# etheriqa/amber

Hardware: AMD Instinct MI355X
Metric: Mrays/sec + wall-clock, Cornell 1024^2 @1024spp; 1/2/4/8 GPU (higher is better)
Workload: dtype f32

## Files before the change

### amber_amd/api.py

```python
from __future__ import annotations

import ctypes as C
import os
import subprocess
from pathlib import Path

import numpy as np

_ROOT = Path(__file__).resolve().parent
_LIB_PATH = _ROOT / "lib" / os.environ.get("AMBER_AMD_LIB", "libamber_hip.so")
_lib = None


class AmberError(RuntimeError):
    """Raised for every non-zero return code of the C ABI (message = amber_hip_last_error())."""


class FlatObject(C.Structure):
    _fields_ = [("kind", C.c_uint32), ("material", C.c_uint32), ("p", C.c_float * 12)]


class FlatMaterial(C.Structure):
    _fields_ = [("kind", C.c_uint32), ("rho", C.c_float * 3), ("param", C.c_float), ("r0", C.c_float)]

# ... 51 lines not shown
class Photon(C.Structure):
    _fields_ = [("pos", C.c_float * 3), ("object", C.c_int32), ("dir_out", C.c_float * 3), ("path", C.c_uint32),
                ("weight", C.c_float * 3), ("sample", C.c_uint32), ("normal", C.c_float * 3), ("bounce", C.c_uint32)]


class PhotonInfo(C.Structure):
    _fields_ = [("n_photons", C.c_uint64), ("n_written", C.c_uint64), ("n_rays", C.c_uint64), ("n_launches", C.c_uint32), ("n_repeats", C.c_uint32)]


class AccumulateInfo(C.Structure):
    _fields_ = [("n_launches", C.c_uint32), ("n_repeats", C.c_uint32), ("rec_count", C.c_uint32), ("flag_words_set", C.c_uint32),
                ("flags_dirty", C.c_uint32)]


LT_SPLAT_CAPACITY0 = 65536
SPLAT_DTYPE = np.dtype([("path", np.uint32), ("sample", np.uint32), ("bounce", np.uint32), ("pixel", np.uint32), ("rgb", np.float32, (3,)), ("pad", np.uint32)])
PHOTON_DIFFUSE, PHOTON_SPECULAR, PHOTON_LIGHT, PHOTON_EYE, PHOTON_ALL = 1, 2, 4, 8, 15
PHOTONS_HOST = 1
PHOTON_CAPACITY0 = 65536
PHOTON_DTYPE = np.dtype([("pos", np.float32, (3,)), ("object", np.int32), ("dir_out", np.float32, (3,)), ("path", np.uint32),
                         ("weight", np.float32, (3,)), ("sample", np.uint32), ("normal", np.float32, (3,)), ("bounce", np.uint32)])


class Ray(C.Structure):
    _fields_ = [("origin", C.c_float * 3), ("t_max", C.c_float), ("dir", C.c_float * 3), ("pad", C.c_uint32)]


class RayHit(C.Structure):
    _fields_ = [("t", C.c_float), ("object", C.c_int32), ("pos", C.c_float * 3), ("normal", C.c_float * 3)]


class PathRay(C.Structure):
    _fields_ = [("origin", C.c_float * 3), ("pad0", C.c_uint32), ("dir", C.c_float * 3), ("pad1", C.c_uint32),
                ("weight", C.c_float * 3), ("pad2", C.c_uint32), ("rng_state", C.c_uint64), ("pad3", C.c_uint64)]


class PathResult(C.Structure):
    _fields_ = [("rgb", C.c_float * 3), ("casts", C.c_uint32), ("rng_state", C.c_uint64), ("pad", C.c_uint32 * 2)]


class AovPixel(C.Structure):
    _fields_ = [("albedo", C.c_float * 3), ("depth", C.c_float), ("normal", C.c_float * 3), ("coverage", C.c_float)]


class DenoiseParams(C.Structure):
    _fields_ = [("levels", C.c_uint32), ("k_normal", C.c_float), ("k_albedo", C.c_float), ("k_depth", C.c_float), ("k_color", C.c_float),
                ("reserved", C.c_uint32 * 3)]


class MomentsPixel(C.Structure):
    _fields_ = [("m1", C.c_float), ("m2", C.c_float), ("batches", C.c_float), ("pad", C.c_float)]


class DenoiseVarianceParams(C.Structure):
    _fields_ = [("levels", C.c_uint32), ("k_normal", C.c_float), ("k_albedo", C.c_float), ("k_depth", C.c_float), ("k_lum", C.c_float),
                ("var_radius", C.c_uint32), ("reserved", C.c_uint32 * 2)]


class TemporalParams(C.Structure):
    _fields_ = [("levels", C.c_uint32), ("max_history", C.c_uint32), ("k_normal", C.c_float), ("k_albedo", C.c_float), ("k_depth", C.c_float),
                ("k_color", C.c_float), ("reserved", C.c_uint32 * 2)]


class HistoryPixel(C.Structure):
    _fields_ = [("color", C.c_float * 3), ("length", C.c_float), ("m1", C.c_float), ("m2", C.c_float), ("pad", C.c_float * 2)]


class BvhDumpInfo(C.Structure):
    _fields_ = [("n_nodes", C.c_uint32), ("n_prims", C.c_uint32), ("root", C.c_int32), ("depth", C.c_uint32),
                ("gmin", C.c_float * 3), ("step", C.c_float * 3), ("reach", C.c_float * 3)]


class HostStats(C.Structure):
    _fields_ = [("rays", C.c_uint64), ("passes", C.c_uint64), ("launches", C.c_uint32), ("pad", C.c_uint32), ("kernel_ms", C.c_double)]


PRIM_TRIANGLE, PRIM_SPHERE, PRIM_DISK, PRIM_CYLINDER = 0, 1, 2, 3
_RECORD = np.dtype([("kind", np.uint32), ("material", np.uint32), ("p", np.float32, (12,))])
MAT_LAMBERTIAN, MAT_PHONG, MAT_SPECULAR, MAT_REFRACTION, MAT_DIFFUSE_LIGHT, MAT_EYE = 0, 1, 2, 3, 4, 5
ENGINE_AUTO, ENGINE_LIST, ENGINE_TWO_PHASE, ENGINE_BVH, ENGINE_WAVEFRONT = 0, 1, 2, 3, 4
ENGINE_REFERENCE_BVH = 6
PT_FLAG_NULL_STREAM, PT_FLAG_BVH_POOL, PT_FLAG_BVH_ITEMS = 1, 2, 4
PT_FLAG_DEVICE_BUILD = 8
BUILD_NONE, BUILD_HOST, BUILD_DEVICE, BUILD_HOST_FALLBACK = 0, 1, 2, 3
BUILD_REASON_NONE, BUILD_REASON_DEPTH, BUILD_REASON_WIDE, BUILD_REASON_BOUNDS = 0, 1, 2, 3
RAYS_HOST = 1
_RAY = np.dtype([("origin", np.float32, (3,)), ("t_max", np.float32), ("dir", np.float32, (3,)), ("pad", np.uint32)])
_RAY_HIT = np.dtype([("t", np.float32), ("object", np.int32), ("pos", np.float32, (3,)), ("normal", np.float32, (3,))])
_PATH_RAY = np.dtype([("origin", np.float32, (3,)), ("pad0", np.uint32), ("dir", np.float32, (3,)), ("pad1", np.uint32),
                      ("weight", np.float32, (3,)), ("pad2", np.uint32), ("rng_state", np.uint64), ("pad3", np.uint64)])
_PATH_RESULT = np.dtype([("rgb", np.float32, (3,)), ("casts", np.uint32), ("rng_state", np.uint64), ("pad", np.uint32, (2,))])
RESOLVE_MEAN_F32, RESOLVE_RGB8, RESOLVE_RGBA8 = 0, 1, 2
RESOLVE_HOST, RESOLVE_MIRROR_X = 1, 2
UPDATE_REFIT, UPDATE_REBUILD = 0, 1

ABI_SYMBOLS = [
    "amber_hip_pt_create", "amber_hip_pt_render_pass", "amber_hip_pt_clear", "amber_hip_pt_sync",
    "amber_hip_pt_download", "amber_hip_pt_device_framebuffer", "amber_hip_pt_stream", "amber_hip_pt_local_rows", "amber_hip_pt_kernel_time", "amber_hip_pt_build_info", "amber_hip_pt_update_objects", "amber_hip_pt_update_lens",
    "amber_hip_pt_cast_rays", "amber_hip_pt_occluded", "amber_hip_pt_resolve", "amber_hip_pt_destroy",
    "amber_hip_pt_trace_paths", "amber_hip_sampler_state",
    "amber_hip_pt_aov_pass", "amber_hip_pt_aov_clear", "amber_hip_pt_aov_download", "amber_hip_pt_device_aov", "amber_hip_pt_denoise",
    "amber_hip_pt_render_batch", "amber_hip_pt_moments_clear", "amber_hip_pt_moments_download", "amber_hip_pt_device_moments", "amber_hip_pt_denoise_variance",
    "amber_hip_pt_temporal", "amber_hip_pt_temporal_reset", "amber_hip_pt_history_download", "amber_hip_pt_device_history",
    "amber_hip_last_error", "amber_hip_abi_version", "amber_hip_math_mode", "amber_hip_device_count", "amber_hip_lt_trace", "amber_hip_lt_trace_range", "amber_hip_lt_render_pass",
    "amber_hip_lt_trace_photons",
    "amber_host_cornell_box", "amber_host_scene_import", "amber_host_scene_create", "amber_host_scene_destroy", "amber_host_scene_flatten",
    "amber_host_pt_create", "amber_host_render", "amber_host_render_devices", "amber_host_last_error", "amber_host_tonemap", "amber_host_export",
]
LAB_SYMBOLS = [
    "amber_hip_kat_cast", "amber_hip_kat_sample", "amber_hip_kat_eye", "amber_hip_kat_trace", "amber_hip_kat_math", "amber_hip_kat_signatures", "amber_hip_pt_signatures",
    "amber_hip_kat_traversal_rate", "amber_hip_kat_pixel_masks", "amber_hip_kat_bvh_dump", "amber_hip_kat_division",
    "amber_hip_kat_sqrt", "amber_hip_kat_sqrt_sweep", "amber_hip_kat_lt_accumulate", "amber_hip_kat_lt_stage_ms",
    "amber_hip_kat_photon_stage_ms",
    "amber_hip_kat_light_ray", "amber_hip_kat_lens_response", "amber_hip_kat_radiance", "amber_host_kat_scene_lights",
    "amber_hip_kat_accumulate", "amber_hip_kat_phase_a",
]
PRODUCT_LIB, LAB_LIB = "libamber_hip.so", "libamber_hip_lab.so"


def library_path() -> Path:
    return _LIB_PATH


def build_library(force: bool = False) -> Path:
    import shutil
    if shutil.which(os.environ.get("HIPCC", "hipcc")) or not _LIB_PATH.exists():
        subprocess.run(["make", "-C", str(_ROOT / "csrc")] + (["-B"] if force else []), check=True)
    return _LIB_PATH


def is_lab() -> bool:
    return hasattr(load_library(), "amber_hip_kat_cast")


def load_library() -> C.CDLL:
    global _lib
    if _lib is not None:
        return _lib
    if not _LIB_PATH.exists():
        raise AmberError(f"{_LIB_PATH} is missing: build it with `make -C amber_amd/csrc` "
                         "(or __graft_entry__.build()); amber_amd has no CPU fallback")
    lib = C.CDLL(str(_LIB_PATH))
    vp, u32, u64, i32 = C.c_void_p, C.c_uint32, C.c_uint64, C.c_int32
    lib.amber_hip_last_error.restype = C.c_char_p
    lib.amber_host_last_error.restype = C.c_char_p
    lib.amber_hip_pt_create.argtypes = [C.POINTER(FlatSceneC), C.POINTER(Sensor), C.POINTER(PtParams), C.POINTER(vp)]
    lib.amber_hip_pt_render_pass.argtypes = [vp, u32, u32]
    lib.amber_hip_pt_clear.argtypes = [vp]
    lib.amber_hip_pt_sync.argtypes = [vp]
    lib.amber_hip_pt_download.argtypes = [vp, vp, C.POINTER(u64)]
    lib.amber_hip_pt_device_framebuffer.argtypes = [vp, C.POINTER(vp), C.POINTER(u64)]
    lib.amber_hip_pt_local_rows.argtypes = [vp, C.POINTER(u32)]
    lib.amber_hip_pt_stream.argtypes = [vp, C.POINTER(vp)]
    lib.amber_hip_pt_kernel_time.argtypes = [vp, C.POINTER(u32), C.POINTER(C.c_double)]
    lib.amber_hip_pt_destroy.argtypes = [vp]
    lib.amber_hip_pt_destroy.restype = None
    if hasattr(lib, "amber_hip_pt_build_info"):
        lib.amber_hip_pt_build_info.argtypes = [vp, C.POINTER(BuildInfo)]
    if hasattr(lib, "amber_hip_pt_update_objects"):
        lib.amber_hip_pt_update_objects.argtypes = [vp, u32, u32, vp, u32, C.POINTER(UpdateInfo)]
    if hasattr(lib, "amber_hip_pt_update_lens"):
        lib.amber_hip_pt_update_lens.argtypes = [vp, C.POINTER(FlatThinLens), vp, u32, C.POINTER(UpdateInfo)]
    if hasattr(lib, "amber_hip_pt_cast_rays"):
        lib.amber_hip_pt_cast_rays.argtypes = [vp, u64, vp, vp, u32]
        lib.amber_hip_pt_occluded.argtypes = [vp, u64, vp, vp, u32]
    if hasattr(lib, "amber_hip_pt_trace_paths"):
        lib.amber_hip_pt_trace_paths.argtypes = [vp, u64, vp, vp, u32, u32, u32]
        lib.amber_hip_sampler_state.argtypes = [u64, u32, u32]
        lib.amber_hip_sampler_state.restype = u64
    if hasattr(lib, "amber_hip_pt_resolve"):
        lib.amber_hip_pt_resolve.argtypes = [vp, u32, u32, vp, u64, u32]
    if hasattr(lib, "amber_hip_pt_aov_pass"):
        lib.amber_hip_pt_aov_pass.argtypes = [vp, u32, u32]
        lib.amber_hip_pt_aov_clear.argtypes = [vp]
        lib.amber_hip_pt_aov_download.argtypes = [vp, vp]
        lib.amber_hip_pt_device_aov.argtypes = [vp, C.POINTER(vp), C.POINTER(u64)]
    if hasattr(lib, "amber_hip_pt_denoise"):
        lib.amber_hip_pt_denoise.argtypes = [vp, u32, C.POINTER(DenoiseParams), u32, vp, u64, u32]
    if hasattr(lib, "amber_hip_pt_render_batch"):
        lib.amber_hip_pt_render_batch.argtypes = [vp, u32, u32]
        lib.amber_hip_pt_moments_clear.argtypes = [vp]
        lib.amber_hip_pt_moments_download.argtypes = [vp, vp]
        lib.amber_hip_pt_device_moments.argtypes = [vp, C.POINTER(vp), C.POINTER(u64)]
        lib.amber_hip_pt_denoise_variance.argtypes = [vp, u32, C.POINTER(DenoiseVarianceParams), u32, vp, u64, u32]
    if hasattr(lib, "amber_hip_pt_temporal"):
        lib.amber_hip_pt_temporal.argtypes = [vp, u32, C.POINTER(TemporalParams), u32, vp, u64, u32]
        lib.amber_hip_pt_temporal_reset.argtypes = [vp]
        lib.amber_hip_pt_history_download.argtypes = [vp, vp]
        lib.amber_hip_pt_device_history.argtypes = [vp, C.POINTER(vp), C.POINTER(u64)]
    if hasattr(lib, "amber_hip_lt_trace"):
        lib.amber_hip_lt_trace.argtypes = [vp, u32, u32, vp, u32, C.POINTER(u32), C.POINTER(u64)]
    if hasattr(lib, "amber_hip_lt_trace_range"):
        lib.amber_hip_lt_trace_range.argtypes = [vp, u32, u32, u32, u32, vp, u32, C.POINTER(u32), C.POINTER(u64)]
    if hasattr(lib, "amber_hip_lt_render_pass"):
        lib.amber_hip_lt_render_pass.argtypes = [vp, u32, u32, C.POINTER(LtPassInfo)]
        if hasattr(lib, "amber_hip_lt_trace_photons"):
            lib.amber_hip_lt_trace_photons.argtypes = [vp, u32, u32, u32, u32, u32, vp, u64, C.POINTER(PhotonInfo), u32]
        if hasattr(lib, "amber_hip_kat_photon_stage_ms"):
            lib.amber_hip_kat_photon_stage_ms.argtypes = [vp, C.POINTER(C.c_double), C.POINTER(C.c_double), C.POINTER(C.c_double)]
    if hasattr(lib, "amber_hip_kat_cast"):
        if hasattr(lib, "amber_hip_kat_phase_a"):
            lib.amber_hip_kat_phase_a.argtypes = [vp, u32, vp, vp, i32, vp, u64, C.POINTER(C.c_uint32)]
        lib.amber_hip_kat_cast.argtypes = [vp, u32, vp, vp, vp, vp, vp, vp]
        lib.amber_hip_kat_sample.argtypes = [vp, u32, vp, vp, vp, vp, vp, vp]
        lib.amber_hip_kat_eye.argtypes = [vp, u32, vp, vp, vp]
        lib.amber_hip_kat_trace.argtypes = [vp, u32, vp, vp, u32, vp, vp]
        lib.amber_hip_kat_math.argtypes = [i32, i32, u32, vp, vp]
        lib.amber_hip_kat_signatures.argtypes = [vp, u32, u32, vp]
        lib.amber_hip_kat_pixel_masks.argtypes = [vp, vp, vp, C.POINTER(C.c_uint32), C.POINTER(C.c_double)]
        lib.amber_hip_kat_traversal_rate.argtypes = [vp, u32, vp, vp, u32, u32, u32, vp, vp, C.POINTER(C.c_double), vp]
        lib.amber_hip_pt_signatures.argtypes = [vp, u32, u32, vp]
        lib.amber_hip_kat_bvh_dump.argtypes = [vp, vp, u32, vp, u32, C.POINTER(BvhDumpInfo)]
        if hasattr(lib, "amber_hip_kat_division"):
            lib.amber_hip_kat_division.argtypes = [i32, i32, u32, vp, vp]
        if hasattr(lib, "amber_hip_kat_sqrt"):
            lib.amber_hip_kat_sqrt.argtypes = [i32, i32, u32, vp, vp]
            lib.amber_hip_kat_sqrt_sweep.argtypes = [i32, u32, u64, C.POINTER(SqrtSweep)]
        if hasattr(lib, "amber_hip_kat_lt_accumulate"):
            lib.amber_hip_kat_lt_accumulate.argtypes = [vp, vp, u32]
            lib.amber_hip_kat_lt_stage_ms.argtypes = [vp, C.POINTER(C.c_double), C.POINTER(C.c_double)]
        if hasattr(lib, "amber_hip_kat_light_ray"):
            lib.amber_hip_kat_light_ray.argtypes = [vp, u32, vp, vp, vp, vp, vp]
            lib.amber_hip_kat_lens_response.argtypes = [vp, u32, vp, vp, vp, vp, vp]
            lib.amber_hip_kat_radiance.argtypes = [vp, u32, vp, vp, vp, vp]
            lib.amber_host_kat_scene_lights.argtypes = [vp, C.POINTER(FlatLight), C.POINTER(u32)]
        if hasattr(lib, "amber_hip_kat_accumulate"):
            lib.amber_hip_kat_accumulate.argtypes = [vp, u32, vp, vp, u32, u32, u32, u64, C.POINTER(AccumulateInfo)]
    lib.amber_host_cornell_box.restype = vp
    lib.amber_host_cornell_box.argtypes = [C.c_float, C.c_float, u32]
    lib.amber_host_scene_import.restype = vp
    lib.amber_host_scene_import.argtypes = [C.c_char_p]
    lib.amber_host_scene_create.restype = vp
    lib.amber_host_scene_create.argtypes = [C.POINTER(FlatObject), u32, C.POINTER(FlatMaterial), u32, C.POINTER(C.c_float),
                                            C.c_float, C.c_float, C.c_float, u32, C.c_int]
    lib.amber_host_scene_destroy.argtypes = [vp]
    lib.amber_host_scene_destroy.restype = None
    lib.amber_host_scene_flatten.argtypes = [vp, C.POINTER(FlatObject), C.POINTER(u32), C.POINTER(FlatMaterial), C.POINTER(u32),
                                             C.POINTER(FlatThinLens)]
    lib.amber_host_pt_create.argtypes = [vp, C.POINTER(Sensor), C.POINTER(PtParams), C.POINTER(vp)]
    lib.amber_host_render.argtypes = [vp, C.c_char_p, C.POINTER(Sensor), u32, u64, u32, C.c_int, u32, vp, C.POINTER(HostStats)]
    lib.amber_host_render_devices.argtypes = [vp, C.c_char_p, C.POINTER(Sensor), u32, u64, u32, C.POINTER(C.c_int), u32, u32, vp, C.POINTER(HostStats)]
    lib.amber_host_tonemap.argtypes = [vp, u32, u32, vp]
    lib.amber_host_export.argtypes = [vp, u32, u32, C.c_char_p, C.c_char_p]
    _lib = lib
    return lib


def _check(rc: int, host: bool = False) -> None:
    if rc != 0:
        lib = load_library()
        msg = (lib.amber_host_last_error() if host else lib.amber_hip_last_error()) or b""
        if host and not msg:
            msg = lib.amber_hip_last_error() or b""
        raise AmberError(f"amber error {rc}: {msg.decode(errors='replace')}")


def device_count() -> int:
    return int(load_library().amber_hip_device_count())


def _f32(a) -> np.ndarray:
    return np.ascontiguousarray(a, dtype=np.float32)


class HostScene:

    def __init__(self, handle):
        if not handle:
            raise AmberError("scene creation failed: " + (load_library().amber_host_last_error() or b"").decode())
        self._h = C.c_void_p(handle)

    @classmethod
    def cornell_box(cls, focal_length: float = 0.050, aperture_radius: float = 0.050, n_blades: int = 6) -> "HostScene":
        return cls(load_library().amber_host_cornell_box(focal_length, aperture_radius, n_blades))

    @classmethod
    def import_file(cls, filename) -> "HostScene":
        return cls(load_library().amber_host_scene_import(str(filename).encode()))

    @classmethod
    def create(cls, objects, materials, transform, focal_length, focus_distance, radius, n_blades, accel: int = 0) -> "HostScene":
        objs = (FlatObject * max(1, len(objects)))()
        for i, (kind, mat, params) in enumerate(objects):
            objs[i].kind, objs[i].material = kind, mat
            for j, v in enumerate(params):
                objs[i].p[j] = v
        mats = (FlatMaterial * max(1, len(materials)))()
        for i, (kind, rho, param) in enumerate(materials):
            mats[i].kind, mats[i].param = kind, param
            for j in range(3):
                mats[i].rho[j] = rho[j]
        t = (C.c_float * 16)(*[float(x) for x in transform])
        return cls(load_library().amber_host_scene_create(objs, len(objects), mats, len(materials), t, focal_length,
                                                          focus_distance, radius, n_blades, accel))

    @classmethod
    def create_arrays(cls, kinds, material_index, params, materials, transform, focal_length, focus_distance, radius, n_blades,
                      accel: int = 0) -> "HostScene":
        n = len(kinds)
        dt = np.dtype([("kind", np.uint32), ("material", np.uint32), ("p", np.float32, (12,))])
        arr = np.zeros(n, dt)
        arr["kind"], arr["material"] = kinds, material_index
        arr["p"][:, : np.asarray(params).shape[1]] = params
        assert arr.itemsize == C.sizeof(FlatObject)
        mats = (FlatMaterial * max(1, len(materials)))()
        for i, (kind, rho, param) in enumerate(materials):
            mats[i].kind, mats[i].param = kind, param
            for j in range(3):
# ... 360 lines not shown

    def device_history(self):
        return self._band_pointer(load_library().amber_hip_pt_device_history)

    def lt_trace(self, first_sample: int, n_samples: int, capacity: int = 1 << 16, paths=None):
        dt = SPLAT_DTYPE
        while True:
            out = np.zeros(capacity, dt)
            n, rays = C.c_uint32(), C.c_uint64()
            if paths is None:
                rc = load_library().amber_hip_lt_trace(self._h, first_sample, n_samples, out.ctypes.data, capacity, C.byref(n), C.byref(rays))
            else:
                rc = load_library().amber_hip_lt_trace_range(self._h, first_sample, n_samples, paths[0], paths[1], out.ctypes.data, capacity,
                                                             C.byref(n), C.byref(rays))
            if rc == -4 and n.value > capacity:
                capacity = n.value
                continue
            _check(rc)
            return out[: n.value], rays.value

    def lt_render_pass(self, first_sample: int, n_samples: int) -> dict:
        info = LtPassInfo()
        _check(load_library().amber_hip_lt_render_pass(self._h, first_sample, n_samples, C.byref(info)))
        return {k: int(getattr(info, k)) for k, _ in LtPassInfo._fields_ if k != "pad"}

    def lt_trace_photons(self, first_sample: int, n_samples: int, surfaces: int = PHOTON_DIFFUSE, paths=None, out=None):
        lib = load_library()
        begin, end = (0, self.sensor.width * self.sensor.height) if paths is None else (int(paths[0]), int(paths[1]))
        info = PhotonInfo()

        def call(ptr, capacity, flags):
            rc = lib.amber_hip_lt_trace_photons(self._h, first_sample, n_samples, begin, end, surfaces, ptr, capacity, C.byref(info), flags)
            d = {k: int(getattr(info, k)) for k, _ in PhotonInfo._fields_}
            if rc != 0:
                try:
                    _check(rc)
                except AmberError as e:
                    e.code, e.info = rc, d
                    raise
            return d

        if out is None:
            need = call(None, 0, PHOTONS_HOST)["n_photons"]
            out = np.zeros(need, PHOTON_DTYPE)
            d = call(out.ctypes.data if need else None, need, PHOTONS_HOST)
            return out, d
        if isinstance(out, np.ndarray):
            if out.dtype != PHOTON_DTYPE or not out.flags.c_contiguous or out.ndim != 1:
                raise AmberError("lt_trace_photons: out must be a contiguous one-dimensional numpy array of PHOTON_DTYPE")
            d = call(out.ctypes.data if len(out) else None, len(out), PHOTONS_HOST)
            return out[: d["n_written"]], d
        if self._is_torch(out):
            import torch
            if not out.is_cuda or not out.is_contiguous() or out.dim() != 2 or out.shape[1] * out.element_size() != 64:
                raise AmberError("lt_trace_photons: out must be a contiguous torch tensor on the handle's device with rows of 64 bytes")
            same = self._torch_enter(torch, out.device)
            try:
                d = call(out.data_ptr() if out.shape[0] else None, out.shape[0], 0)
            finally:
                self._torch_leave(same)
            return out[: d["n_written"]], d
        ptr, capacity = out
        d = call(ptr, capacity, 0)
        return d["n_written"], d

    def kat_photon_stage_ms(self):
        a, b, c = C.c_double(), C.c_double(), C.c_double()
        _check(load_library().amber_hip_kat_photon_stage_ms(self._h, C.byref(a), C.byref(b), C.byref(c)))
        return a.value, b.value, c.value

    def kat_lt_accumulate(self, records) -> None:
        rec = np.ascontiguousarray(records, SPLAT_DTYPE)
        _check(load_library().amber_hip_kat_lt_accumulate(self._h, rec.ctypes.data if len(rec) else None, len(rec)))

    def kat_accumulate(self, n_samples: int, q, rgb, n_waves: int = 4, rec_capacity: int = 0, rays: int = 0) -> dict:
        qq = np.ascontiguousarray(q, np.uint32).reshape(-1)
        cc = _f32(rgb).reshape(-1, 3)
        assert len(qq) == len(cc)
        info = AccumulateInfo()
        _check(load_library().amber_hip_kat_accumulate(self._h, n_samples, qq.ctypes.data if len(qq) else None, cc.ctypes.data if len(qq) else None,
                                                       len(qq), n_waves, rec_capacity, rays, C.byref(info)))
        return {k: int(getattr(info, k)) for k, _ in AccumulateInfo._fields_}

    def kat_lt_stage_ms(self):
        a, b = C.c_double(), C.c_double()
        _check(load_library().amber_hip_kat_lt_stage_ms(self._h, C.byref(a), C.byref(b)))
        return a.value, b.value

    def kat_cast(self, origins, dirs):
        o, d = _f32(origins).reshape(-1, 3), _f32(dirs).reshape(-1, 3)
        n = len(o)
        obj, t = np.empty(n, np.int32), np.empty(n, np.float32)
        pos, nrm = np.empty((n, 3), np.float32), np.empty((n, 3), np.float32)
        _check(load_library().amber_hip_kat_cast(self._h, n, o.ctypes.data, d.ctypes.data, obj.ctypes.data, t.ctypes.data,
                                                 pos.ctypes.data, nrm.ctypes.data))
        return obj, t, pos, nrm

    def kat_phase_a(self, origins, dirs, axis_loops: bool = True):
        o, d = _f32(origins).reshape(-1, 3), _f32(dirs).reshape(-1, 3)
        n = len(o)
        out, groups = np.zeros(4 * n, np.uint32), C.c_uint32()
        _check(load_library().amber_hip_kat_phase_a(self._h, n, o.ctypes.data, d.ctypes.data, int(bool(axis_loops)), out.ctypes.data, out.size, C.byref(groups)))
        return out[:n * groups.value].reshape(n, groups.value)

    def kat_sample(self, material, normals, dirs_out, rng_state, importance: bool = False):
        m = np.ascontiguousarray(material, np.uint32) | np.uint32(0x80000000 if importance else 0)
        nn, dd = _f32(normals).reshape(-1, 3), _f32(dirs_out).reshape(-1, 3)
        st = np.ascontiguousarray(rng_state, np.uint64).copy()
        n = len(m)
        di, w = np.empty((n, 3), np.float32), np.empty((n, 3), np.float32)
        _check(load_library().amber_hip_kat_sample(self._h, n, m.ctypes.data, nn.ctypes.data, dd.ctypes.data, st.ctypes.data,
                                                   di.ctypes.data, w.ctypes.data))
        return di, w, st

    def kat_eye(self, pixel, sample):
        p, s = np.ascontiguousarray(pixel, np.uint32), np.ascontiguousarray(sample, np.uint32)
        out = np.empty((len(p), 7), np.float32)
        _check(load_library().amber_hip_kat_eye(self._h, len(p), p.ctypes.data, s.ctypes.data, out.ctypes.data))
        return out

    def kat_light_ray(self, rng_state):
        st = np.ascontiguousarray(rng_state, np.uint64).copy()
        n = len(st)
        o, d, w = np.empty((n, 3), np.float32), np.empty((n, 3), np.float32), np.empty((n, 3), np.float32)
        light = np.empty(n, np.uint32)
        _check(load_library().amber_hip_kat_light_ray(self._h, n, st.ctypes.data, o.ctypes.data, d.ctypes.data, w.ctypes.data, light.ctypes.data))
        return o, d, w, light, st

    def kat_lens_response(self, position, direction_out):
        p, d = _f32(position).reshape(-1, 3), _f32(direction_out).reshape(-1, 3)
        n = len(p)
        reached, pixel, value = np.empty(n, np.uint32), np.empty(n, np.uint32), np.empty(n, np.float32)
        _check(load_library().amber_hip_kat_lens_response(self._h, n, p.ctypes.data, d.ctypes.data, reached.ctypes.data, pixel.ctypes.data,
                                                          value.ctypes.data))
        return reached, pixel, value

    def kat_radiance(self, material, normals, dirs_out):
        m = np.ascontiguousarray(material, np.uint32)
        nn, dd = _f32(normals).reshape(-1, 3), _f32(dirs_out).reshape(-1, 3)
        out = np.empty((len(m), 3), np.float32)
        _check(load_library().amber_hip_kat_radiance(self._h, len(m), m.ctypes.data, nn.ctypes.data, dd.ctypes.data, out.ctypes.data))
        return out

    def kat_trace(self, pixel, sample, max_bounces: int = 16):
        p, s = np.ascontiguousarray(pixel, np.uint32), np.ascontiguousarray(sample, np.uint32)
        rec = np.zeros((len(p), max_bounces, 11), np.uint32)
        casts = np.zeros(len(p), np.uint32)
        _check(load_library().amber_hip_kat_trace(self._h, len(p), p.ctypes.data, s.ctypes.data, max_bounces, rec.ctypes.data,
                                                  casts.ctypes.data))
        return rec, casts

    def kat_traversal_rate(self, origins, dirs, waves: int = 5, refill_min: int = 16, repeats: int = 3, rounds=None):
        o, d = _f32(origins).reshape(-1, 3), _f32(dirs).reshape(-1, 3)
        n = len(o)
        obj, t, ms = np.empty(n, np.int32), np.empty(n, np.float32), C.c_double()
        _check(load_library().amber_hip_kat_traversal_rate(self._h, n, o.ctypes.data, d.ctypes.data, waves, refill_min, repeats, t.ctypes.data,
                                                           obj.ctypes.data, C.byref(ms), rounds.ctypes.data if rounds is not None else None))
        return obj, t, ms.value

    def kat_signatures(self, first_sample: int, n_samples: int) -> np.ndarray:
        rows, width, _ = self.band_shape
        out = np.zeros((rows, width, n_samples), np.uint64)
        _check(load_library().amber_hip_kat_signatures(self._h, first_sample, n_samples, out.ctypes.data))
        return out

    def pixel_masks(self):
# ... 95 lines not shown
```

### amber_amd/csrc/hip/dev_shading.h

```cpp
#pragma once

namespace amber_dev {

__device__ __forceinline__ V3 PerfectReflection(V3 incident, V3 normal, float signed_cos) {
  return (2.0f * signed_cos) * normal - incident;
}
__device__ __forceinline__ V3 HemispherePSA(V3 w, uint64_t& rng) {
  V3 u, v; OrthonormalBasis(w, u, v);
  const float r0 = Uniform(rng);
  const float r1 = Uniform(rng);
  const float cos_theta = Sqrt(r0);
  const float sin_theta = Sqrt(1.0f - r0);
  const float phi = 2.0f * 3.14159274f * r1;
  float sp, cp; SinCos(phi, sp, cp);
  return u * sin_theta * cp + v * sin_theta * sp + w * cos_theta;
}
__device__ __forceinline__ V3 CosinePower(V3 w, float exponent, uint64_t& rng) {
  V3 u, v; OrthonormalBasis(w, u, v);
  const float r0 = Uniform(rng);
  const float r1 = Uniform(rng);
  const float cos_theta = Pow(r0, 1.0f / (exponent + 1.0f));
  const float sin_theta = Sqrt(1.0f - cos_theta * cos_theta);
  const float phi = 2.0f * 3.14159274f * r1;
  float sp, cp; SinCos(phi, sp, cp);
// ... 87 lines not shown
  const float rho_t = 1.0f - rho_r;
  const float p_r = (rho_r + 0.5f) / 2.0f;
  const float p_t = (rho_t + 0.5f) / 2.0f;
  const bool reflect = Uniform(rng) < p_r;
  dir_in = reflect ? dir_r : dir_t;
  weight = ((reflect ? rho_r : rho_t) / (reflect ? p_r : p_t)) * rho;
}

__device__ __forceinline__ void GenerateLightRay(const DevScene& sc, uint64_t& rng, V3& origin, V3& dir, V3& weight, int& origin_slot) {
  const float x = Uniform(rng) * sc.total_power;
  uint32_t pos = 0;
  while (pos + 1u < sc.n_lights && sc.lights[pos].cum_power < x) ++pos;
  const DevLight* L = sc.lights + pos;
  const uint32_t kind = L->kind;
  V3 normal;
  if (kind == PRIM_TRIANGLE) {
    float u = Uniform(rng), v = Uniform(rng);
    if (u + v >= 1.0f) { u = 1.0f - u; v = 1.0f - v; }
    origin = (1.0f - u - v) * ld3(L->p) + u * ld3(L->p + 3) + v * ld3(L->p + 6);
    normal = ld3(L->p + 9);
  } else if (kind == PRIM_SPHERE) {
    const float r0 = Uniform(rng) * (1.0f - (-1.0f)) + (-1.0f);
    const float r1 = Uniform(rng);
    const float sin_theta = Sqrt(1.0f - r0 * r0);
    float sp, cp; SinCos(2.0f * 3.14159274f * r1, sp, cp);
    normal = v3(r0 * cp, r0 * sp, sin_theta);
    origin = ld3(L->p) + L->p[3] * normal;
  } else if (kind == PRIM_DISK) {
    const float radius = Sqrt(Uniform(rng) * (L->p[6] * L->p[6]));
    const V3 N = ld3(L->p + 3);
    V3 u, v; OrthonormalBasis(N, u, v);
    float ay, ax; SinCos(Uniform(rng) * 6.28318548f, ay, ax);
    origin = ld3(L->p) + (u * ax + v * ay) * radius;
    normal = N;
  } else {
    const float height = Uniform(rng) * L->p[7];
    const V3 N = ld3(L->p + 3);
    V3 u, v; OrthonormalBasis(N, u, v);
    float ay, ax; SinCos(Uniform(rng) * 6.28318548f, ay, ax);
    const V3 n = u * ax + v * ay;
    origin = ld3(L->p) + N * height + n * L->p[6];
    normal = Normalize(n);
  }
  dir = HemispherePSA(normal, rng);
  weight = ld3(L->irr) / L->pdf_area;
  origin_slot = L->slot;
}

__device__ __forceinline__ DevLens LoadLens(const DevLens* lens) {
  ConstWords w = (ConstWords)(lens);
  asm volatile("" : "+s"(w));
  union { DevLens lens; uint32_t words[sizeof(DevLens) / 4]; } u;
#pragma unroll
  for (unsigned k = 0; k < sizeof(DevLens) / 4; ++k) u.words[k] = w[k];
  return u.lens;
}
__device__ __forceinline__ DevLens LoadLens(const DevScene& sc) { return LoadLens(sc.lens); }

__device__ __forceinline__ bool LensResponse(const DevScene& sc, V3 position, V3 direction_out, uint32_t& pixel, float& value) {
  const DevLens L = LoadLens(sc);
  const V3 direction = MatMul(L.local_, direction_out);
  float sx, sy;
  if (L.kind == 1u) {
    const V3 point = (L.sensor_distance / direction.z) * direction;
    sx = point.x; sy = point.y; value = 1.0f;
  } else {
    if (direction.z >= 0.0f) return false;
    const V3 aperture_point = MatMul(L.local_, position - ld3(L.origin));
    const V3 sensor_point = L.neg_sd_over_fd * aperture_point + (L.sensor_distance / direction.z) * direction;
    sx = sensor_point.x; sy = sensor_point.y;
    value = static_cast<float>(Pow4(Normalize(sensor_point - aperture_point).z / direction.z));
  }
  const float uvx = sx / sc.sensor.sw + 0.5f, uvy = sy / sc.sensor.sh + 0.5f;
  const float mn = uvy < uvx ? uvy : uvx, mx = uvx < uvy ? uvy : uvx;
  if (mn < 0.0f || mx >= 1.0f) return false;
  uint32_t ix = static_cast<uint32_t>(uvx * sc.sensor.wf), iy = static_cast<uint32_t>(uvy * sc.sensor.hf);
  if (ix > sc.sensor.w - 1u) ix = sc.sensor.w - 1u;
  if (iy > sc.sensor.h - 1u) iy = sc.sensor.h - 1u;
  pixel = ix + iy * sc.sensor.w;
  return true;
}

struct EyeRayScene { const DevLens* lens; const DevBlade* blades; DevSensor sensor; };
template <bool kSharedDiv = false, int kSqrt = SQRT_PLAIN, typename Scene>
__device__ __forceinline__ void GenerateEyeRay(const Scene& sc, uint32_t px, uint32_t py, uint64_t& rng,
                                               V3& origin, V3& dir, float& weight, int& origin_slot, bool* near_edge = nullptr) {
  const DevLens L = LoadLens(sc.lens);
  if (L.kind == 1u) {
    const float jy = Uniform(rng);
    const float jx = Uniform(rng);
    const float uvx = (static_cast<float>(px) + jx) / sc.sensor.wf;
    const float uvy = (static_cast<float>(py) + jy) / sc.sensor.hf;
    const V3 sensor_point = v3((uvx - 0.5f) * sc.sensor.sw, (uvy - 0.5f) * sc.sensor.sh, L.sensor_distance);
    const V3 ray_dir = Normalize<kSharedDiv, kSqrt>(MatMul(L.global_, -sensor_point));
    const V3 dl = MatMul(L.local_, ray_dir);
    const V3 point = (L.sensor_distance / dl.z) * dl;
    const float geometry_factor = dl.z * dl.z / SquaredLength(point);
    const float pdf_dir = L.inv_scene_area / geometry_factor;
    origin = ld3(L.origin); dir = ray_dir;
    weight = 1.0f / 1.0f / pdf_dir;
    origin_slot = -1;
    if (near_edge) *near_edge = true;
    return;
  }
  const float fpos = __builtin_floorf(Uniform(rng) * L.n_blades_f);
  uint32_t pos = static_cast<uint32_t>(fpos);
  if (pos > L.n_blades - 1) pos = L.n_blades - 1;
  const DevBlade* bl = sc.blades + pos;
  float u = Uniform(rng);
  float v = Uniform(rng);
  if (u + v >= 1.0f) { u = 1.0f - u; v = 1.0f - v; }
  if (near_edge) *near_edge = !(u >= L.edge_tol && v >= L.edge_tol && u + v <= 1.0f - L.edge_tol);
  const V3 ap_origin = (1.0f - u - v) * ld3(bl->v0) + u * ld3(bl->v1) + v * ld3(bl->v2);
  const V3 aperture_point = MatMul(L.local_, ap_origin - ld3(L.origin));
  const float jy = Uniform(rng);
  const float jx = Uniform(rng);
  const float uvx = (static_cast<float>(px) + jx) / sc.sensor.wf;
  const float uvy = (static_cast<float>(py) + jy) / sc.sensor.hf;
  const V3 sensor_point = v3((uvx - 0.5f) * sc.sensor.sw, (uvy - 0.5f) * sc.sensor.sh, L.sensor_distance);
  const V3 direction = Normalize<kSharedDiv, kSqrt>(L.neg_fd_over_sd * sensor_point - aperture_point);
  const double factor = Pow4(Normalize<false, kSqrt>(sensor_point - aperture_point).z / direction.z);
  const V3 ray_dir = Normalize<kSharedDiv, kSqrt>(MatMul(L.global_, direction));
  const V3 dloc = MatMul(L.local_, ray_dir);
  const float pdf_dir = static_cast<float>(static_cast<double>(L.size_over_area) * L.sd2 / Pow4(dloc.z));
  origin = ap_origin; dir = ray_dir;
  origin_slot = bl->slot;
  weight = static_cast<float>(factor / static_cast<double>(L.p_area) / static_cast<double>(pdf_dir));
}

struct Bounce { int object; float t; V3 pos; V3 weight_before; };

struct SplatSink { DevSplat* records; unsigned int* count; uint32_t capacity; uint32_t path, sample; float size_f; };

enum { SINK_SPLATS = 0, SINK_PHOTONS = 1 };
struct PhotonSink : SplatSink { float4* photons; uint32_t surfaces; };
#ifndef AMBER_PHOTON_CLAIM_PER_LANE
#define AMBER_PHOTON_CLAIM_PER_LANE 0
#endif

template <bool kTrace, int kEngine, bool kLight, bool kDivBasis = false, bool kDivHit = false, uint32_t kSqrtMask = 0u, int kSink = SINK_SPLATS>
__device__ __forceinline__ bool PathShade(const DevScene& sc, const DevObject* lds_objects, const HitRec& h, V3& o, V3& d, V3& weight, V3& measurement,
                                          uint64_t& rng, uint32_t& casts, int& origin_slot, Bounce* trace AMBER_STAMP_PARAM, const SplatSink* sink);

template <bool kTrace, int kEngine, bool kLight = false, bool kDivBasis = false, bool kDivHit = false, uint32_t kSqrtMask = 0u, int kSink = SINK_SPLATS>
__device__ __forceinline__ bool PathStep(const DevScene& sc, const DevObject* lds_objects, int32_t* lds_stack, V3& o, V3& d, V3& weight, V3& measurement,
                                         uint64_t& rng, uint32_t& casts, int& origin_slot, Bounce* trace AMBER_STAMP_PARAM, const SplatSink* sink = nullptr,
                                         const bool use_premask = false, const uint32_t premask = 0u, const int bvh_stack_cap = AMBER_BVH_STACK) {
  HitRec h;
  ClosestHit<kEngine, (kSqrtMask & 8u) ? SQRT_EXACT : SQRT_PLAIN>(sc, lds_objects, lds_stack, o, d, origin_slot, h AMBER_STAMP_ARG, use_premask, premask, bvh_stack_cap);
  return PathShade<kTrace, kEngine, kLight, kDivBasis, kDivHit, kSqrtMask, kSink>(sc, lds_objects, h, o, d, weight, measurement, rng, casts, origin_slot, trace AMBER_STAMP_ARG, sink);
}

template <bool kTrace, int kEngine, bool kLight, bool kDivBasis, bool kDivHit, uint32_t kSqrtMask, int kSink>
__device__ __forceinline__ bool PathShade(const DevScene& sc, const DevObject* lds_objects, const HitRec& h, V3& o, V3& d, V3& weight, V3& measurement,
                                          uint64_t& rng, uint32_t& casts, int& origin_slot, Bounce* trace AMBER_STAMP_PARAM, const SplatSink* splat_sink) {
  casts++;
  if (h.idx < 0) {
    if (kTrace) { trace->object = -1; trace->t = __builtin_nanf(""); trace->pos = v3(0, 0, 0); trace->weight_before = v3(0, 0, 0); }
    return false;
  }
  V3 pos, normal; uint32_t mat;
  ResolveHit<kEngine, kDivHit>(sc, lds_objects, h, o, d, pos, normal, mat);
  const DevMaterial m = sc.materials[mat];
  const V3 dir_out = -d;
  if (kTrace) { trace->object = h.idx; trace->t = h.t; trace->pos = pos; trace->weight_before = weight; }
  V3 dir_in, sw;
  if (kLight) {
    if (kSink == SINK_PHOTONS) {
      const PhotonSink* const sink = static_cast<const PhotonSink*>(splat_sink);
      const bool rec = ((0x842211u >> (m.kind * 4u)) & sink->surfaces) != 0u;
#if !AMBER_PHOTON_CLAIM_PER_LANE
      const unsigned long long voters = __ballot(rec);
#endif
      if (rec) {
#if AMBER_PHOTON_CLAIM_PER_LANE
        const unsigned int k = atomicAdd(sink->count, 1u);
#else
        const uint32_t rank = __builtin_amdgcn_mbcnt_hi(static_cast<uint32_t>(voters >> 32), __builtin_amdgcn_mbcnt_lo(static_cast<uint32_t>(voters), 0u));
        unsigned int base = 0u;
        if (rank == 0u) base = atomicAdd(sink->count, static_cast<unsigned int>(__popcll(voters)));
        const unsigned int k = static_cast<unsigned int>(__builtin_amdgcn_readlane(static_cast<int>(base), __builtin_ctzll(voters))) + rank;
#endif
        if (k < sink->capacity) {
          float4* const r = sink->photons + static_cast<size_t>(k) * 4u;
          r[0] = make_float4(pos.x, pos.y, pos.z, __int_as_float(h.idx));
          r[1] = make_float4(dir_out.x, dir_out.y, dir_out.z, __uint_as_float(sink->path));
          r[2] = make_float4(weight.x, weight.y, weight.z, __uint_as_float(sink->sample));
          r[3] = make_float4(normal.x, normal.y, normal.z, __uint_as_float(casts));
        }
      }
    } else if (m.kind == MAT_EYE) {
      const SplatSink* const sink = splat_sink;
      uint32_t pixel; float value;
      if (LensResponse(sc, pos, dir_out, pixel, value)) {
        const V3 add = (weight * value) / sink->size_f;
        const unsigned int k = atomicAdd(sink->count, 1u);
        if (k < sink->capacity) {
          DevSplat& r = sink->records[k];
          r.path = sink->path; r.sample = sink->sample; r.bounce = casts; r.pixel = pixel;
          r.rgb[0] = add.x; r.rgb[1] = add.y; r.rgb[2] = add.z; r.pad = 0u;
        }
      }
    }
    AMBER_STAMP(4);
    SampleImportance(m, normal, dir_out, rng, dir_in, sw);
  } else {
    measurement = measurement + weight * Radiance(m, normal, dir_out);
    AMBER_STAMP(4);
    SampleLight<kDivBasis, kSqrtMask>(m, normal, dir_out, rng, dir_in, sw);
  }
  AMBER_STAMP(5);
  float p_rr = 0.9375f;
  const float mw = Max3(sw);
  if (mw < p_rr) p_rr = mw;
  if (Uniform(rng) >= p_rr) return false;
  if (sc.max_depth && casts >= sc.max_depth) return false;
  o = pos; d = dir_in;
  if (kEngine == ENGINE_TWO_PHASE_N) origin_slot = (lds_objects[h.slot].kind & 0x80u) ? h.slot : -1;
  else origin_slot = (kEngine == ENGINE_TWO_PHASE && static_cast<uint32_t>(h.slot) < sc.n_prog_tris) ? h.slot : -1;
#if AMBER_SHARED_WEIGHT_QUOTIENT
  {
    const uint32_t bx = __float_as_uint(sw.x), by = __float_as_uint(sw.y), bz = __float_as_uint(sw.z);
    const float qx = sw.x / p_rr;
    float qy = by == bx ? qx : 0.0f, qz = bz == bx ? qx : 0.0f;
    const bool hard_y = !(by == bx || (by == 0u && p_rr > 0.0f)), hard_z = !(bz == bx || (bz == 0u && p_rr > 0.0f));
    if (__ballot(hard_y || hard_z) != 0ull) {
      if (hard_y) qy = sw.y / p_rr;
      if (hard_z) qz = sw.z / p_rr;
    }
    weight = weight * v3(qx, qy, qz);
  }
#else
  weight = weight * (sw / p_rr);
#endif
  return true;
}

}
```

### amber_amd/csrc/hip/lab_api.inc

```

namespace {
constexpr const char* kKatNoRefBvh = "the known-answer kernels have no instantiation for AMBER_ENGINE_REFERENCE_BVH (its traversal stack belongs to the render kernels' grid): compare amber_hip_pt_signatures instead";
template <typename F>
void WithKatEngine(const amber_hip_pt* h, F&& f) {
  WithHitEngine(h->hit_engine, [&](auto engine) -> int { if constexpr (decltype(engine)::value != ENGINE_REF_BVH) f(engine); return AMBER_OK; });
}

int RenderPassWavefront(amber_hip_pt* h, uint32_t first_sample, uint32_t n_samples) {
  const uint32_t n_pixels = static_cast<uint32_t>(BandPixels(h));
  const uint64_t kMaxPaths = 1ull << 28;
  uint64_t max_chunks = kMaxPaths / (static_cast<uint64_t>(n_pixels) * AMBER_ACCUM_CHUNK);
  if (max_chunks == 0) return Fail(AMBER_EINVAL, "band too large for the wavefront engine");
  const uint32_t kMaxBounces = 4096;
  const uint64_t cap = max_chunks * AMBER_ACCUM_CHUNK;
  return SplitSamples(first_sample, n_samples, "band too large for the wavefront engine", [&](uint32_t left, amber_plan::Launch* l) -> int {
    *l = {left > cap ? static_cast<uint32_t>(cap) : left, 0};
    return AMBER_OK;
  }, [&](uint32_t first, const amber_plan::Launch& l, bool*) -> int {
    const uint32_t n = l.n;
    const uint32_t n_chunks = (n + AMBER_ACCUM_CHUNK - 1) / AMBER_ACCUM_CHUNK;
    const size_t n_paths = static_cast<size_t>(n_chunks) * n_pixels * AMBER_ACCUM_CHUNK;
    const size_t shard_capacity = ((n_paths + AMBER_WF_SHARDS - 1) / AMBER_WF_SHARDS + 63) / 64 * 64 + 64;
    const size_t q_len = shard_capacity * AMBER_WF_SHARDS;
    const size_t n_counts = static_cast<size_t>(kMaxBounces + 2) * AMBER_WF_SHARDS;
// ... 349 lines not shown
  if (n > kMaxPathsPerLaunch) return Fail(AMBER_EINVAL, "too many paths for one call");
  HIP_TRY(hipSetDevice(h->device));
  AMBER_TRY(ResolvePending(h));
  HIP_TRY(hipStreamSynchronize(h->stream));
  AMBER_TRY(Grow(h, h->d_sig, n, "signatures"));
  HIP_TRY(hipMemsetAsync(h->d_sig, 0, n * sizeof(unsigned long long), h->stream));
  AMBER_TRY(RenderSamples(h, first_sample, n_samples, n_pixels, h->d_fb, h->d_sig));
  HIP_TRY(hipStreamSynchronize(h->stream));
  HIP_TRY(hipMemcpy(out, h->d_sig, n * sizeof(uint64_t), hipMemcpyDeviceToHost));
  return AMBER_OK;
}); }

int amber_hip_kat_lt_accumulate(amber_hip_pt* h, const AmberSplat* records, uint32_t n) { return Guarded("amber_hip_kat_lt_accumulate", [&]() -> int {
  if (!h || (n && !records)) return Fail(AMBER_EINVAL, "null argument");
  if (!WholeFrame(h)) return Fail(AMBER_EINVAL, "amber_hip_kat_lt_accumulate: the handle renders a band or stripes of the frame");
  if (n > 0x7fffffffu) return Fail(AMBER_EINVAL, "too many records for one call");
  const uint32_t npx = h->scene.sensor.w * h->scene.sensor.h;
  for (uint32_t i = 0; i < n; i++) if (records[i].pixel >= npx) return Fail(AMBER_EINVAL, "pixel index out of range");
  if (n == 0) return AMBER_OK;
  HIP_TRY(hipSetDevice(h->device));
  AMBER_TRY(ResolvePending(h));
  AMBER_TRY(EnsureLtSplats(h, n));
  static_assert(sizeof(AmberSplat) == sizeof(DevSplat), "splat layouts must agree");
  HIP_TRY(hipMemcpyAsync(h->d_splats, records, static_cast<size_t>(n) * sizeof(DevSplat), hipMemcpyHostToDevice, h->stream));
  HIP_TRY(hipMemsetAsync(h->lt.longest.p, 0, sizeof(unsigned int), h->stream));
  AMBER_TRY(LtAccumulate(h, n, 32u));
  HIP_TRY(hipStreamSynchronize(h->stream));
  return AMBER_OK;
}); }

int amber_hip_kat_accumulate(amber_hip_pt* h, uint32_t n_samples, const uint32_t* q, const float* rgb, uint32_t n_items, uint32_t n_waves, uint32_t rec_capacity,
                             uint64_t rays, AmberAccumulateInfo* info) { return Guarded("amber_hip_kat_accumulate", [&]() -> int {
  if (info) *info = AmberAccumulateInfo{};
  if (!h || (n_items && (!q || !rgb))) return Fail(AMBER_EINVAL, "null argument");
  if (n_samples == 0 || n_waves == 0) return Fail(AMBER_EINVAL, "amber_hip_kat_accumulate: n_samples and n_waves must not be zero");
  if (n_waves > (1u << 20)) return Fail(AMBER_EINVAL, "amber_hip_kat_accumulate: more than 2^20 waves");
  const uint64_t n_paths = BandPixels(h) * n_samples;
  if (n_paths >= (1ull << 32)) return Fail(AMBER_EINVAL, "amber_hip_kat_accumulate: n_pixels * n_samples must stay below 2^32");
  {
    std::vector<uint32_t> seen;
    seen.reserve(n_items);
    for (uint32_t i = 0; i < n_items; i++) {
      if (q[i] == AMBER_REC_UNUSED) continue;
      if (q[i] >= n_paths) return Fail(AMBER_EINVAL, "amber_hip_kat_accumulate: item " + std::to_string(i) + ": path index out of range");
      seen.push_back(q[i]);
    }
    std::sort(seen.begin(), seen.end());
    if (std::adjacent_find(seen.begin(), seen.end()) != seen.end()) return Fail(AMBER_EINVAL, "amber_hip_kat_accumulate: a path index occurs twice");
  }
  HIP_TRY(hipSetDevice(h->device));
  AMBER_TRY(ResolvePending(h));
  PathLaunchBufs& p = h->paths;
  if (rec_capacity != 0 && rec_capacity < p.rec_capacity)
    return Fail(AMBER_EINVAL, "amber_hip_kat_accumulate: rec_capacity " + std::to_string(rec_capacity) + " is below the " + std::to_string(p.rec_capacity) + " slots the handle's record buffer has");
  const uint32_t n_pixels = static_cast<uint32_t>(BandPixels(h));
  if (n_pixels == 0) return AMBER_OK;
  AMBER_TRY(EnsureRecordCapacity(h, rec_capacity ? rec_capacity : static_cast<uint64_t>(n_items) + RecordSlack(h)));
  DevBuf<uint32_t> d_q; DevBuf<float> d_rgb;
  HIP_TRY(d_q.alloc(n_items ? n_items : 1u)); HIP_TRY(d_rgb.alloc(n_items ? 3ull * n_items : 1u));
  if (n_items) {
    HIP_TRY(hipMemcpy(d_q.p, q, 4ull * n_items, hipMemcpyHostToDevice));
    HIP_TRY(hipMemcpy(d_rgb.p, rgb, 12ull * n_items, hipMemcpyHostToDevice));
  }
  RecordProducer producer;
  producer.lab = true; producer.q = d_q.p; producer.rgb = d_rgb.p; producer.n_items = n_items; producer.n_waves = n_waves; producer.rays = rays;
  const uint64_t launches0 = p.n_launches, repeats0 = p.n_repeats;
  AMBER_TRY(LaunchLabRecords(h, n_samples, n_pixels, h->d_fb, producer));
  const int rc = ResolvePending(h);
  p.pending = false; p.pending_producer = RecordProducer{};
  AMBER_TRY(rc);
  const size_t used_words = static_cast<size_t>((n_paths + 31u) / 32u);
  std::vector<uint32_t> words(used_words);
  if (used_words) HIP_TRY(hipMemcpyAsync(words.data(), p.flags, used_words * sizeof(uint32_t), hipMemcpyDeviceToHost, h->stream));
  HIP_TRY(hipStreamSynchronize(h->stream));
  if (info) {
    info->n_launches = static_cast<uint32_t>(p.n_launches - launches0); info->n_repeats = static_cast<uint32_t>(p.n_repeats - repeats0);
    info->rec_count = *p.h_rec_count.v;
    info->flag_words_set = static_cast<uint32_t>(std::count_if(words.begin(), words.end(), [](uint32_t w) { return w != 0u; }));
    info->flags_dirty = p.flags_dirty ? 1u : 0u;
  }
  return AMBER_OK;
}); }

int amber_hip_kat_lt_stage_ms(amber_hip_pt* h, double* sort_ms, double* sum_ms) { return Guarded("amber_hip_kat_lt_stage_ms", [&]() -> int {
  if (!h) return Fail(AMBER_EINVAL, "null handle");
  h->lt.stage_timing = true;
  if (sort_ms) *sort_ms = h->lt.sort_ms;
  if (sum_ms) *sum_ms = h->lt.sum_ms;
  h->lt.sort_ms = h->lt.sum_ms = 0;
  return AMBER_OK;
}); }

int amber_hip_kat_photon_stage_ms(amber_hip_pt* h, double* trace_ms, double* sort_ms, double* gather_ms) { return Guarded("amber_hip_kat_photon_stage_ms", [&]() -> int {
  if (!h) return Fail(AMBER_EINVAL, "null handle");
  PhotonBufs& s = h->photons;
  s.stage_timing = true;
  if (trace_ms) *trace_ms = s.trace_ms;
  if (sort_ms) *sort_ms = s.sort_ms;
  if (gather_ms) *gather_ms = s.gather_ms;
  s.trace_ms = s.sort_ms = s.gather_ms = 0;
  return AMBER_OK;
}); }

int amber_hip_kat_math(int device, int mode, uint32_t n, const float* x, float* out) { return Guarded("amber_hip_kat_math", [&]() -> int {
  if (!x || !out || mode < 0 || mode > 3) return Fail(AMBER_EINVAL, "bad argument");
  if (n == 0) return AMBER_OK;
  int n_dev = 0;
  if (hipGetDeviceCount(&n_dev) != hipSuccess || device < 0 || device >= n_dev) return Fail(AMBER_ENODEVICE, "no such HIP device");
  HIP_TRY(hipSetDevice(device));
  const size_t n_in = mode == 1 ? 2ull * n : n, n_out = mode == 1 ? n : 2ull * n;
  DevBuf<float> d_x, d_o;
  HIP_TRY(d_x.alloc(n_in)); HIP_TRY(d_o.alloc(n_out));
  HIP_TRY(hipMemcpy(d_x.p, x, n_in * 4, hipMemcpyHostToDevice));
  hipLaunchKernelGGL(kat_math_kernel, dim3((n + 255) / 256), dim3(256), 0, 0, mode, n, d_x.p, d_o.p);
  HIP_TRY(hipGetLastError());
  HIP_TRY(hipDeviceSynchronize());
  HIP_TRY(hipMemcpy(out, d_o.p, n_out * 4, hipMemcpyDeviceToHost));
  return AMBER_OK;
}); }

int amber_hip_kat_division(int device, int mode, uint32_t n, const float* x, float* out) { return Guarded("amber_hip_kat_division", [&]() -> int {
  if (!x || !out || mode < 0 || mode > 3) return Fail(AMBER_EINVAL, "bad argument");
  if (n == 0) return AMBER_OK;
  if (n > 0x3fffffffu) return Fail(AMBER_EINVAL, "too many groups for one call");
  int n_dev = 0;
  if (hipGetDeviceCount(&n_dev) != hipSuccess || device < 0 || device >= n_dev) return Fail(AMBER_ENODEVICE, "no such HIP device");
  HIP_TRY(hipSetDevice(device));
  DevBuf<float> d_x, d_o;
  HIP_TRY(d_x.alloc(4ull * n)); HIP_TRY(d_o.alloc(3ull * n));
  HIP_TRY(hipMemcpy(d_x.p, x, 16ull * n, hipMemcpyHostToDevice));
  hipLaunchKernelGGL(kat_division_kernel, dim3((n + 255) / 256), dim3(256), 0, 0, mode, n, d_x.p, d_o.p);
  HIP_TRY(hipGetLastError());
  HIP_TRY(hipDeviceSynchronize());
  HIP_TRY(hipMemcpy(out, d_o.p, 12ull * n, hipMemcpyDeviceToHost));
  return AMBER_OK;
}); }

int amber_hip_kat_sqrt(int device, int mode, uint32_t n, const float* x, float* out) { return Guarded("amber_hip_kat_sqrt", [&]() -> int {
  if (!x || !out || mode < 0 || mode > 4) return Fail(AMBER_EINVAL, "bad argument");
  if (n == 0) return AMBER_OK;
  if (n > 0x3fffffffu) return Fail(AMBER_EINVAL, "too many items for one call");
  int n_dev = 0;
  if (hipGetDeviceCount(&n_dev) != hipSuccess || device < 0 || device >= n_dev) return Fail(AMBER_ENODEVICE, "no such HIP device");
  HIP_TRY(hipSetDevice(device));
  const size_t width = mode <= 1 ? 1u : (mode <= 3 ? 3u : 2u);
  DevBuf<float> d_x, d_o;
  HIP_TRY(d_x.alloc(width * n)); HIP_TRY(d_o.alloc(width * n));
  HIP_TRY(hipMemcpy(d_x.p, x, width * n * 4, hipMemcpyHostToDevice));
  hipLaunchKernelGGL(kat_sqrt_kernel, dim3((n + 255) / 256), dim3(256), 0, 0, mode, n, d_x.p, d_o.p);
  HIP_TRY(hipGetLastError());
  HIP_TRY(hipDeviceSynchronize());
  HIP_TRY(hipMemcpy(out, d_o.p, width * n * 4, hipMemcpyDeviceToHost));
  return AMBER_OK;
}); }

int amber_hip_kat_sqrt_sweep(int device, uint32_t first_bits, uint64_t count, AmberSqrtSweep* out) { return Guarded("amber_hip_kat_sqrt_sweep", [&]() -> int {
  if (!out || count == 0 || static_cast<uint64_t>(first_bits) + count > (1ull << 32)) return Fail(AMBER_EINVAL, "bad argument");
  int n_dev = 0;
  if (hipGetDeviceCount(&n_dev) != hipSuccess || device < 0 || device >= n_dev) return Fail(AMBER_ENODEVICE, "no such HIP device");
  HIP_TRY(hipSetDevice(device));
  static_assert(sizeof(SqrtSweepCounters) == sizeof(AmberSqrtSweep), "the kernel's counters are the C record");
  DevBuf<SqrtSweepCounters> d_c;
  HIP_TRY(d_c.alloc(1));
  HIP_TRY(hipMemset(d_c.p, 0, sizeof(SqrtSweepCounters)));
  const uint64_t blocks = (count + 255u) / 256u;
  hipLaunchKernelGGL(kat_sqrt_sweep_kernel, dim3(static_cast<uint32_t>(blocks < 8192u ? blocks : 8192u)), dim3(256), 0, 0, first_bits, static_cast<unsigned long long>(count), d_c.p);
// ... 8 lines not shown
```

### amber_amd/csrc/hip/pt_args.h

```cpp
#pragma once

struct RenderArgs {
  DevScene scene;
  float* partial;
  uint32_t* flags;
  uint32_t* touched;
  uint4* records;
  unsigned int* rec_count;
  uint32_t rec_capacity;
  unsigned long long* ray_count;
  unsigned int* next_item;
  unsigned long long* stamps;
  DevSplat* splats;
  unsigned int* splat_count;
  uint32_t splat_capacity;
  uint32_t photon_surfaces;
  int32_t* bvh_stack;
  float* carried;
  const uint32_t* pixel_mask;
  unsigned long long* sig;
  uint64_t hashed_seed;
  uint32_t row_begin;
  uint32_t stripe_rows, stripe_period;
  ExactDiv div_stripe_rows;
  ExactDiv div_width;
  uint32_t n_pixels;
  uint32_t first_sample, n_samples;
  uint32_t n_chunks, n_items;
  ExactDiv div_samples;
  uint32_t path_offset;
  uint32_t shade_batch;

  void SetBand(uint32_t row_begin_, uint32_t stripe_rows_, uint32_t stripe_period_) {
    row_begin = row_begin_; stripe_rows = stripe_rows_; stripe_period = stripe_period_;
    div_stripe_rows = MakeExactDiv(stripe_rows_); div_width = MakeExactDiv(scene.sensor.w);
  }
  void SetSamples(uint32_t first_sample_, uint32_t n_samples_) { first_sample = first_sample_; n_samples = n_samples_; div_samples = MakeExactDiv(n_samples_); }
};

template <bool kPhotons>
__device__ __forceinline__ typename std::conditional<kPhotons, PhotonSink, SplatSink>::type MakeLightSink(const RenderArgs& a, uint32_t path, uint32_t sample) {
  const SplatSink splat{a.splats, a.splat_count, a.splat_capacity, path, sample, a.scene.sensor.size_f};
  if constexpr (kPhotons) return PhotonSink{splat, reinterpret_cast<float4*>(a.splats), a.photon_surfaces};
  else return splat;
}

__device__ __forceinline__ uint32_t FrameRow(uint32_t row_begin, uint32_t stripe_rows, uint32_t stripe_period, ExactDiv div_stripe_rows, uint32_t lrow) {
  if (stripe_rows == 0u) return row_begin + lrow;
  const uint32_t band = Quotient(div_stripe_rows, lrow);
  return row_begin + band * stripe_period + (lrow - band * stripe_rows);
}

struct ColdArgs {
  ConstWords w;
  __device__ __forceinline__ static ColdArgs Open() {
    ConstWords w = (ConstWords)__builtin_amdgcn_kernarg_segment_ptr();
    asm volatile("" : "+s"(w));
    return ColdArgs{w};
  }
  template <typename T> __device__ __forceinline__ T Get(size_t byte_offset) const {
    static_assert(sizeof(T) % 4 == 0 && alignof(T) <= 8, "whole dwords");
    union U { T value; uint32_t words[sizeof(T) / 4]; __device__ U() {} } u;
#pragma unroll
    for (unsigned k = 0; k < sizeof(T) / 4; ++k) u.words[k] = w[byte_offset / 4 + k];
    return u.value;
  }
};
#define AMBER_COLD(cold, field) (cold).Get<decltype(static_cast<const RenderArgs*>(nullptr)->field)>(offsetof(RenderArgs, field))

__device__ __forceinline__ uint32_t Fnv32(uint32_t h, uint32_t v) {
#pragma unroll
  for (int k = 0; k < 4; k++) { h ^= (v >> (8 * k)) & 0xffu; h *= 16777619u; }
  return h;
}

#define AMBER_REC_BLOCK 64u
#define AMBER_REC_UNUSED 0xffffffffu
struct RecordSink { uint4* records; uint32_t* flags; uint32_t* touched; unsigned int* rec_count; uint32_t rec_capacity; ExactDiv div_samples; };
template <typename SinkOf>
__device__ __forceinline__ void EmitRecords(SinkOf sink_of, bool emit, uint32_t q, V3 meas, uint32_t& rec_next, uint32_t& rec_end) {
  const unsigned long long me = __ballot(emit);
  if (me == 0ull) return;
  const RecordSink a = sink_of();
  const uint32_t n = static_cast<uint32_t>(__popcll(me));
  const uint32_t rank = __builtin_amdgcn_mbcnt_hi(static_cast<uint32_t>(me >> 32), __builtin_amdgcn_mbcnt_lo(static_cast<uint32_t>(me), 0u));
  const uint32_t room = rec_end - rec_next;
  uint32_t fresh = 0;
  if (n > room) {
    if ((threadIdx.x & 63u) == 0u) fresh = atomicAdd(a.rec_count, AMBER_REC_BLOCK);
    fresh = __builtin_amdgcn_readfirstlane(fresh);
  }
  if (emit) {
    const uint32_t slot = rank < room ? rec_next + rank : fresh + (rank - room);
    if (slot < a.rec_capacity) a.records[slot] = make_uint4(q, __float_as_uint(meas.x), __float_as_uint(meas.y), __float_as_uint(meas.z));
    atomicOr(a.flags + (q >> 5), 1u << (q & 31u));
    const uint32_t p = Quotient(a.div_samples, q);
    atomicOr(a.touched + (p >> 5), 1u << (p & 31u));
  }
  if (n > room) { rec_next = fresh + (n - room); rec_end = fresh + AMBER_REC_BLOCK; }
  else rec_next += n;
}
__device__ __forceinline__ void EmitRecords(const RenderArgs& a, bool emit, uint32_t q, V3 meas, uint32_t& rec_next, uint32_t& rec_end) {
  EmitRecords([&]() { return RecordSink{a.records, a.flags, a.touched, a.rec_count, a.rec_capacity, a.div_samples}; }, emit, q, meas, rec_next, rec_end);
}
__device__ __forceinline__ void CloseRecords(const RenderArgs& a, uint32_t rec_next, uint32_t rec_end) {
  const uint32_t k = rec_next + (threadIdx.x & 63u);
  if (k < rec_end && k < a.rec_capacity) a.records[k].x = AMBER_REC_UNUSED;
}
```

### amber_amd/csrc/hip/pt_device.h

```cpp
#pragma once

#include <hip/hip_runtime.h>
#include <stdint.h>

#include "dev_scene.h"
#include "shared_div.h"
#include "exact_sqrt.h"
#include "dev_math.h"
#include "dev_primitives.h"
#include "dev_two_phase.h"
#include "dev_bvh.h"
#include "dev_closest_hit.h"
#include "dev_shading.h"
```

### amber_amd/csrc/hip/pt_host.hip

```cpp
#include <hip/hip_runtime.h>
#include <rocprim/device/device_radix_sort.hpp>
#include <rocprim/device/device_scan.hpp>

#include <algorithm>
#include <chrono>
#include <cmath>
#include <cstdio>
#include <cstdlib>
#include <cstring>
#include <memory>
#include <string>
#include <type_traits>
#include <utility>
#include <vector>

#include "../../../include/amber_hip.h"
#ifdef AMBER_LAB
#include "../../../include/amber_hip_lab.h"
#endif
#include "c_boundary.h"
#include "pt_device.h"
#include "exact_div.h"
#include "launch_plan.h"
#include "bvh_build.h"
#include "filter_build.h"
#include "ref_bvh_build.h"

using namespace amber_dev;

namespace {

#include "pt_args.h"
#include "pt_megakernel.inc"
#include "pt_records.inc"
#include "pt_bvh_megakernel.inc"
#ifdef AMBER_LAB
#include "bvh_pool.inc"
#include "bvh_stream.inc"
#include "wavefront.inc"
#include "lab_kernels.inc"
#endif

template <typename T>
struct DevBuf {
  T* p = nullptr;
  size_t n = 0;
  DevBuf() = default;
  DevBuf(DevBuf&& o) noexcept : p(o.p), n(o.n) { o.p = nullptr; o.n = 0; }
  ~DevBuf() { reset(); }
  void reset() { if (p) (void)hipFree(p); p = nullptr; n = 0; }
  hipError_t alloc(size_t count) {
    reset();
    const hipError_t e = hipMalloc(&p, (count ? count : 1) * sizeof(T));
    if (e != hipSuccess) p = nullptr; else n = count;
    return e;
  }
  void swap(DevBuf& o) noexcept { std::swap(p, o.p); std::swap(n, o.n); }
  hipError_t need(size_t count) {
    if (p && n >= count) return hipSuccess;
    DevBuf bigger;
    const hipError_t e = bigger.alloc(count);
    if (e == hipSuccess) swap(bigger);
    return e;
  }
  operator T*() const { return p; }
};
template <typename T, auto kRelease>
struct Owned {
  T v{};
  Owned() = default;
  Owned(Owned&& o) noexcept : v(o.v) { o.v = T{}; }
  ~Owned() { if (v) (void)kRelease(v); }
};
using Event = Owned<hipEvent_t, hipEventDestroy>;

}

#include "scene_prep.h"
using amber_prep::kHitTwoPhaseN;

namespace {
namespace dbuild { struct Reduced; }
struct BvhTreeBufs { DevBuf<uint8_t> nodes, prims, tris, objects, spheres; };
struct BvhBuildScratch {
  DevBuf<dbuild::Reduced> red; DevBuf<amber_bvh::Box> boxes; DevBuf<unsigned long long> codes, codes_sorted; DevBuf<uint32_t> index, sorted; DevBuf<uint8_t> temp;
  DevBuf<int32_t> left, right; DevBuf<uint32_t> first, last, parent_node, parent_object, child_boxes, arrivals, live, rank;
  DevBuf<AmberFlatObject> staged;
  DevBuf<uint32_t> refit_parent;
  bool refit_parent_valid = false;
  DevBuf<double> area;
  DevBuf<uint8_t> retired_nodes;
};
struct LtAccumBufs {
  DevBuf<unsigned long long> key[2];
  DevBuf<uint32_t> index[2];
  DevBuf<float4> value;
  DevBuf<uint8_t> temp;
  DevBuf<unsigned int> longest;
  uint32_t capacity = 0;
#ifdef AMBER_LAB
  bool stage_timing = false;
  double sort_ms = 0, sum_ms = 0;
  Event ev[3];
#endif
};
struct PhotonBufs {
  DevBuf<float4> staging;
  uint32_t capacity = 0;
  DevBuf<unsigned int> count;
  DevBuf<unsigned long long> rays;
  DevBuf<float4> sorted;
#ifdef AMBER_LAB
  bool stage_timing = false;
  double trace_ms = 0, sort_ms = 0, gather_ms = 0;
  Event ev[5];
#endif
};
// ... 17 lines not shown
  DevBuf<unsigned int> next;
  DevBuf<float4> rays;
  DevBuf<uint8_t> out;
};
struct RecordProducer {
  bool lab = false;
  const uint32_t* q = nullptr;
  const float* rgb = nullptr;
  uint32_t n_items = 0, n_waves = 0;
  unsigned long long rays = 0;
};
struct PathLaunchBufs {
  DevBuf<uint32_t> flags;  bool flags_dirty = true;
  DevBuf<uint32_t> touched;
  DevBuf<uint4> records;   DevBuf<float> sorted;   uint32_t rec_capacity = 0;
  DevBuf<unsigned int> launch_ctl;
  unsigned int* rec_count = nullptr;
  unsigned long long* rays_launch = nullptr;
  DevBuf<uint32_t> excl, block_sum;
  Owned<unsigned int*, hipHostFree> h_rec_count;
  Event pending_event;
  bool pending = false, pending_checked = true;
  uint32_t pending_first = 0, pending_n = 0;
  float* pending_target = nullptr;
  RecordProducer pending_producer;
  uint64_t n_launches = 0, n_repeats = 0;
  bool density_known = false;
  double rec_density = 0;
  DevBuf<float> carried;
};
struct LaunchTimer {
  std::vector<std::pair<Event, Event>> events;
  size_t used = 0;
  uint32_t folded_launches = 0;
  double folded_ms = 0;
  void reset() { used = 0; folded_launches = 0; folded_ms = 0; }
};
}

struct amber_hip_pt : amber_prep::SceneState {
  int device = 0;
  Owned<hipStream_t, hipStreamDestroy> own_stream;
  hipStream_t stream = nullptr;
  amber_prep::EnvSwitches env;
  std::vector<DevBuf<uint8_t>> scene_arrays;
  DevBuf<uint8_t> objects_buf;
  BvhTreeBufs tree;
  DevBuf<uint8_t> objects_alt;
  BvhBuildScratch update_scratch;
  uint32_t create_flags = 0;
  size_t n_triangles = 0;
  bool has_spheres = false;
  uint32_t small_kinds[3] = {0, 0, 0};
  uint32_t first_blade = 0;
  std::vector<AmberFlatObject> blade_records;
  DevBuf<uint8_t> lens_alt[2];
  uint32_t lens_alt_next = 0;
  std::vector<uint8_t> lens_stage;
  std::vector<uint32_t> light_object;
  std::vector<float> light_p;
  bool lights_stale = false;
  bool area_known = false;
  float tree_area = 0;
  double area_host[4] = {0, 0, 0, 0};
  DevBuf<uint2> d_ref_stack;
  uint64_t ref_stack_threads = 0;
  RayQueryBufs query;
  ImageStageBufs img;
  DevBuf<float> d_fb;
  DevBuf<unsigned long long> d_rays;
  DevBuf<unsigned int> d_next;
  DevBuf<unsigned long long> d_stamps;
  DevBuf<DevSplat> d_splats;
  DevBuf<unsigned int> d_splat_count;
  uint64_t hashed_seed_lt = 0;
  LtAccumBufs lt;
  PhotonBufs photons;
  DevBuf<float> d_partial;
  PathLaunchBufs paths;
  DevBuf<int32_t> d_bvh_stack;
  DevBuf<unsigned long long> d_sig;
  DevBuf<uint32_t> d_pixel_mask;
  bool pixel_mask_ready = false;
  int n_cus = 256;
  uint32_t row_begin = 0, row_end = 0, stripe_rows = 0, stripe_period = 0, local_rows = 0;
  uint64_t seed = 0, hashed_seed = 0;
  DevBuf<float> d_wf;
  uint32_t n_materials = 0;
  LaunchTimer timer;
};

#include "bvh_device_build.inc"
#include "bvh_update.inc"

namespace {

uint64_t HostSplitMix64(uint64_t z) {
  z += 0x9E3779B97F4A7C15ull;
  z = (z ^ (z >> 30)) * 0xBF58476D1CE4E5B9ull;
  z = (z ^ (z >> 27)) * 0x94D049BB133111EBull;
  return z ^ (z >> 31);
}

int StartPixelMasks(amber_hip_pt* h, float* timing);
uint64_t BandPixels(const amber_hip_pt* h);
uint32_t PersistentBlocks(const amber_hip_pt* h, uint64_t n_items = ~0ull, bool pool = false);

int ValidateScene(const AmberFlatScene* s, const AmberSensor* sensor) {
  if (!s || !sensor) return Fail(AMBER_EINVAL, "null scene or sensor");
  if (!s->objects || s->n_objects == 0) return Fail(AMBER_EINVAL, "scene has no objects");
  if (s->n_objects >= (1u << 26)) return Fail(AMBER_EINVAL, "too many objects (engine BVH addresses its 48-byte leaf records with 32-bit byte offsets: fewer than 2^26 objects)");
  if (!s->materials || s->n_materials == 0) return Fail(AMBER_EINVAL, "scene has no materials");
  if (sensor->width == 0 || sensor->height == 0) return Fail(AMBER_EINVAL, "empty sensor");
  if (static_cast<uint64_t>(sensor->width) * sensor->height >= (1ull << 32)) return Fail(AMBER_EINVAL, "sensor too large");
  for (uint32_t i = 0; i < s->n_objects; i++) {
    if (s->objects[i].kind > AMBER_PRIM_CYLINDER) return Fail(AMBER_EINVAL, "object " + std::to_string(i) + ": unknown primitive kind");
    if (s->objects[i].material >= s->n_materials) return Fail(AMBER_EINVAL, "object " + std::to_string(i) + ": material index out of range");
  }
  for (uint32_t i = 0; i < s->n_materials; i++)
    if (s->materials[i].kind > AMBER_MAT_EYE) return Fail(AMBER_EINVAL, "material " + std::to_string(i) + ": unknown kind");
  if (s->n_lights && !s->lights) return Fail(AMBER_EINVAL, "n_lights > 0 but lights is null");
  for (uint32_t i = 0; i < s->n_lights; i++)
    if (s->lights[i].object >= s->n_objects) return Fail(AMBER_EINVAL, "light object index out of range");
  const AmberFlatThinLens& L = s->lens;
  if (L.n_blades == 0) return Fail(AMBER_EINVAL, "lens has no aperture blades");
  if (L.kind > AMBER_LENS_PINHOLE) return Fail(AMBER_EINVAL, "unknown lens kind");
  if (static_cast<uint64_t>(L.first_blade_object) + L.n_blades > s->n_objects) return Fail(AMBER_EINVAL, "aperture blade objects out of range");
  for (uint32_t i = 0; i < L.n_blades; i++)
    if (s->objects[L.first_blade_object + i].kind != AMBER_PRIM_TRIANGLE) return Fail(AMBER_EINVAL, "aperture blade is not a triangle");
  return AMBER_OK;
}


template <typename T, typename P>
hipError_t UploadTo(DevBuf<uint8_t>& b, const std::vector<T>& v, size_t extra, P& dst) {
  hipError_t e = b.alloc((v.size() + extra) * sizeof(T));
  if (e == hipSuccess && !v.empty()) e = hipMemcpy(b, v.data(), v.size() * sizeof(T), hipMemcpyHostToDevice);
  if (e == hipSuccess) dst = reinterpret_cast<T*>(b.p);
  return e;
}
template <typename T, typename P>
hipError_t Upload(amber_hip_pt* h, const std::vector<T>& v, size_t extra, P& dst) {
  DevBuf<uint8_t> b;
  const hipError_t e = UploadTo(b, v, extra, dst);
  if (e == hipSuccess) h->scene_arrays.push_back(std::move(b));
  return e;
}

int Create(const AmberFlatScene* s, const AmberSensor* sensor, const AmberPtParams* params, amber_hip_pt** out) {
  const auto t_create = std::chrono::steady_clock::now();
  auto ms_since = [](std::chrono::steady_clock::time_point t0) { return std::chrono::duration<double, std::milli>(std::chrono::steady_clock::now() - t0).count(); };
  AMBER_TRY(ValidateScene(s, sensor));
  int n_dev = 0;
  if (hipGetDeviceCount(&n_dev) != hipSuccess || n_dev <= 0)
    return Fail(AMBER_ENODEVICE, "no HIP device available (this engine has no CPU fallback)");
  if (params->device < 0 || params->device >= n_dev) return Fail(AMBER_ENODEVICE, "device ordinal out of range");
  uint32_t rb = params->row_begin, re = params->row_end;
  if (rb == 0 && re == 0) re = sensor->height;
  if (rb > re || re > sensor->height) return Fail(AMBER_EINVAL, "bad row band");
  uint32_t local_rows = re - rb;
  if (params->stripe_rows) {
    if (params->stripe_period < params->stripe_rows) return Fail(AMBER_EINVAL, "stripe_period must be >= stripe_rows");
    const uint32_t q = (re - rb) / params->stripe_period, rem = (re - rb) % params->stripe_period;
    local_rows = q * params->stripe_rows + (rem < params->stripe_rows ? rem : params->stripe_rows);
  }
  if (params->engine > AMBER_ENGINE_REFERENCE_BVH || params->engine == 5u) return Fail(AMBER_EINVAL, "unknown engine");
#ifndef AMBER_LAB
  if (params->engine == AMBER_ENGINE_WAVEFRONT) return Fail(AMBER_EINVAL, "engine WAVEFRONT (the streaming formulation, kept for measurement) is part of the lab build, libamber_hip_lab.so");
  if (params->reserved & AMBER_PT_FLAG_BVH_POOL) return Fail(AMBER_EINVAL, "AMBER_PT_FLAG_BVH_POOL (pt_bvh_pool_kernel, kept for measurement) is part of the lab build, libamber_hip_lab.so");
#endif
  if (params->engine == AMBER_ENGINE_REFERENCE_BVH && !amber_refbvh::CentresAreOrdered(s->objects, s->n_objects))
    return Fail(AMBER_EINVAL, "AMBER_ENGINE_REFERENCE_BVH: an object's centre is NaN (the reference's build sorts objects by centre; std::sort is undefined on NaN keys)");
  if (params->engine == AMBER_ENGINE_TWO_PHASE && s->n_objects > AMBER_MAX_GROUP_OBJECTS)
    return Fail(AMBER_EINVAL, "AMBER_ENGINE_TWO_PHASE supports at most 128 objects");

  HIP_TRY(hipSetDevice(params->device));
  const amber_prep::EnvSwitches env = amber_prep::ReadEnv();
  amber_prep::PreparedScene p = amber_prep::PrepareScene(s, sensor, params, env, AMBER_PATH_BVH_STACK, AMBER_BVH_SHADE_BATCH);
  if (!p.error.empty()) return Fail(AMBER_EINVAL, p.error);

  std::unique_ptr<amber_hip_pt, void (*)(amber_hip_pt*)> h(new amber_hip_pt(), amber_hip_pt_destroy);
  h->device = params->device;
  h->env = env;
  h->row_begin = rb; h->row_end = re; h->local_rows = local_rows;
  h->stripe_rows = params->stripe_rows; h->stripe_period = params->stripe_rows ? params->stripe_period : 0;
  h->seed = params->seed; h->hashed_seed = HostSplitMix64(params->seed);
  h->hashed_seed_lt = HostSplitMix64(params->seed + 0x6C74ull);
  if (params->stream) { h->stream = static_cast<hipStream_t>(params->stream); }
  else if (params->reserved & AMBER_PT_FLAG_NULL_STREAM) { h->stream = nullptr; }
  else {
    hipError_t e = hipStreamCreateWithFlags(&h->own_stream.v, hipStreamNonBlocking);
    if (e != hipSuccess) return Fail(AMBER_EHIP, std::string("hipStreamCreate: ") + hipGetErrorString(e));
    h->stream = h->own_stream.v;
  }
  static_cast<amber_prep::SceneState&>(*h) = std::move(p);
  h->n_materials = s->n_materials;
  { int v = 0; if (hipDeviceGetAttribute(&v, hipDeviceAttributeMultiprocessorCount, params->device) == hipSuccess && v > 0) h->n_cus = v; }

  DevScene& sc = h->scene;
  HIP_TRY(UploadTo(h->objects_buf, p.objects, 0, sc.objects));
  h->create_flags = params->reserved;
  h->n_triangles = amber_prep::CountTriangles(p.objects);
  for (size_t i = 0; i < p.objects.size(); i++) {
    h->has_spheres = h->has_spheres || (p.objects[i].kind & 0xffu) == AMBER_PRIM_SPHERE;
    if (i < 3) h->small_kinds[i] = p.objects[i].kind & 0xffu;
  }
  h->first_blade = s->lens.first_blade_object;
  h->blade_records.assign(s->objects + s->lens.first_blade_object, s->objects + s->lens.first_blade_object + s->lens.n_blades);
  for (uint32_t i = 0; i < s->n_lights; i++) {
    h->light_object.push_back(s->lights[i].object);
    h->light_p.insert(h->light_p.end(), s->objects[s->lights[i].object].p, s->objects[s->lights[i].object].p + 12);
  }
  HIP_TRY(Upload(h.get(), p.materials, 0, sc.materials));
  HIP_TRY(Upload(h.get(), p.blades, 0, sc.blades));
  HIP_TRY(Upload(h.get(), p.planes, 1, sc.planes));
  HIP_TRY(Upload(h.get(), p.tri_filters, 1, sc.tri_filters));
  HIP_TRY(Upload(h.get(), p.sphere_filters, 1, sc.sphere_filters));
  HIP_TRY(Upload(h.get(), p.prog_objects, 1, sc.prog_objects));
  if (!p.groups.empty()) HIP_TRY(Upload(h.get(), p.groups, 0, sc.groups));
  HIP_TRY(Upload(h.get(), p.lights, 1, sc.lights));
  if (p.bvh_pending) {
    const auto t_tree = std::chrono::steady_clock::now();
    uint32_t reason = AMBER_BUILD_REASON_NONE, n_nodes = 0, depth = 0;
    {
      BvhBuildScratch scratch;
      dbuild::BuildInput in{};
      in.objs = sc.objects; in.n = static_cast<uint32_t>(p.objects.size()); in.any_tri = h->n_triangles != 0; in.has_spheres = h->has_spheres;
      in.rmin_known = true; in.rmin = 3.0e38f;
      for (const DevObject& o : p.objects) if ((o.kind & 0xffu) == AMBER_PRIM_SPHERE) in.rmin = std::min(in.rmin, std::fabs(o.radius));
      for (int k = 0; k < 3; k++) in.small_kinds[k] = h->small_kinds[k];
      dbuild::BuildResult res{};
      AMBER_TRY(DeviceBuildBvh(h.get(), in, scratch, &res));
      reason = res.reason; n_nodes = res.n_nodes; depth = res.depth;
    }
    if (reason == AMBER_BUILD_REASON_NONE) {
      amber_prep::ChooseBvhScheduler(*h, p.objects, params, env, n_nodes, depth, AMBER_PATH_BVH_STACK, AMBER_BVH_SHADE_BATCH);
      h->build.where = AMBER_BUILD_DEVICE; h->build.n_nodes = n_nodes; h->build.n_leaves = n_nodes + 1u; h->build.depth = depth;
      p.bvh_pending = false;
      h->build.tree_ms = ms_since(t_tree);
    } else {
      const double spent = ms_since(t_tree);
      amber_prep::HostBvhFallback(*h, p, reason, params, env, AMBER_PATH_BVH_STACK, AMBER_BVH_SHADE_BATCH);
      h->build.tree_ms += spent;
    }
  }
  if (h->build.where != AMBER_BUILD_DEVICE) {
    const auto t_upload = std::chrono::steady_clock::now();
    HIP_TRY(UploadTo(h->tree.nodes, p.bvh_nodes, 1, sc.bvh_nodes));
#if AMBER_BVH_WIDE
    HIP_TRY(Upload(h.get(), p.bvh_nodes4, 1, sc.bvh_nodes4));
#endif
    HIP_TRY(UploadTo(h->tree.prims, p.bvh_prims, 1, sc.bvh_prims));
    HIP_TRY(UploadTo(h->tree.tris, p.bvh_tris, 3, sc.bvh_tris));
    HIP_TRY(UploadTo(h->tree.objects, p.bvh_objects, 1, sc.bvh_objects));
    HIP_TRY(UploadTo(h->tree.spheres, p.bvh_spheres, 1, sc.bvh_spheres));
    if (h->hit_engine == AMBER_ENGINE_BVH) h->build.tree_ms += ms_since(t_upload);
  }
  HIP_TRY(Upload(h.get(), std::vector<DevLens>{p.lens}, 0, sc.lens));
  const size_t fb_floats = static_cast<size_t>(local_rows) * sensor->width * 3;
  HIP_TRY(h->d_fb.alloc(fb_floats));
  HIP_TRY(h->d_rays.alloc(1));
  HIP_TRY(h->d_next.alloc(1));
#ifdef AMBER_STAMPS
  HIP_TRY(h->d_stamps.alloc(8 + 4 * AMBER_WAVE_TIME_SLOTS));
  HIP_TRY(hipMemset(h->d_stamps, 0, (8 + 4 * AMBER_WAVE_TIME_SLOTS) * sizeof(unsigned long long)));
#endif
  HIP_TRY(hipMemsetAsync(h->d_fb, 0, fb_floats * sizeof(float), h->stream));
  HIP_TRY(hipMemsetAsync(h->d_rays, 0, sizeof(unsigned long long), h->stream));
  if (h->hit_engine == AMBER_ENGINE_REFERENCE_BVH) {
    HIP_TRY(Upload(h.get(), p.ref_nodes, 1, sc.ref_nodes));
    HIP_TRY(Upload(h.get(), p.ref_leaves, 1, sc.ref_leaves));
    const uint64_t threads = static_cast<uint64_t>(PersistentBlocks(h.get())) * 256u;
    const uint64_t bytes = threads * (static_cast<uint64_t>(p.ref_depth) + 1u) * sizeof(uint2);
    if (bytes > (64ull << 30)) return Fail(AMBER_ENOMEM, "the reference's BVH of this scene is " + std::to_string(p.ref_depth) + " levels deep: its traversal stacks would take " + std::to_string(bytes >> 30) + " GiB");
    HIP_TRY(h->d_ref_stack.alloc(bytes / sizeof(uint2)));
    sc.ref_stack = h->d_ref_stack; sc.ref_stack_stride = static_cast<uint32_t>(threads); h->ref_stack_threads = threads;
  }
  AMBER_TRY(StartPixelMasks(h.get(), nullptr));
  h->build.create_ms = ms_since(t_create);
  *out = h.release();
  return AMBER_OK;
}

}
// ... 315 lines not shown
```

### amber_amd/csrc/hip/pt_launch.inc

```

namespace {
using amber_plan::kMaxPathsPerLaunch;

template <typename F>
int TimedLaunch(amber_hip_pt* h, bool timed, F&& launch) {
  LaunchTimer& t = h->timer;
  if (timed && t.used == 64) {
    HIP_TRY(hipStreamSynchronize(h->stream));
    for (size_t i = 0; i < t.used; i++) {
      float ms = 0;
      HIP_TRY(hipEventElapsedTime(&ms, t.events[i].first.v, t.events[i].second.v));
      t.folded_ms += ms;
    }
    t.folded_launches += static_cast<uint32_t>(t.used);
    t.used = 0;
  }
  if (timed && t.used == t.events.size()) {
    std::pair<Event, Event> ev;
    HIP_TRY(hipEventCreate(&ev.first.v)); HIP_TRY(hipEventCreate(&ev.second.v));
    t.events.push_back(std::move(ev));
  }
  std::pair<Event, Event>* const ev = timed ? &t.events[t.used++] : nullptr;
  if (ev) HIP_TRY(hipEventRecord(ev->first.v, h->stream));
  AMBER_TRY(launch());
// ... 63 lines not shown
  RenderArgs a{};
  a.scene = h->scene; a.hashed_seed = hashed_seed; a.SetBand(h->row_begin, h->stripe_rows, h->stripe_period); a.n_pixels = n_pixels;
  a.SetSamples(first_sample, n_samples); a.n_chunks = (n_samples + AMBER_ACCUM_CHUNK - 1) / AMBER_ACCUM_CHUNK;
  return a;
}


uint64_t RecordSlack(const amber_hip_pt* h) { return static_cast<uint64_t>(h->n_cus) * 8u * 4u * AMBER_REC_BLOCK + 4096u; }

int EnsureRecordCapacity(amber_hip_pt* h, uint64_t slots) {
  PathLaunchBufs& p = h->paths;
  if (slots <= p.rec_capacity) return AMBER_OK;
  if (slots > 0xfffffff0ull) return Fail(AMBER_ENOMEM, "record buffer beyond 2^32 slots");
  p.rec_capacity = 0;
  AMBER_TRY(Grow(h, p.records, slots, "path records"));
  AMBER_TRY(Grow(h, p.sorted, slots * 3u, "path records"));
  p.rec_capacity = static_cast<uint32_t>(slots);
  return AMBER_OK;
}

int EnsureLaunchCtl(amber_hip_pt* h) {
  PathLaunchBufs& p = h->paths;
  if (!p.launch_ctl) {
    HIP_TRY(p.launch_ctl.alloc(4));
    p.rec_count = p.launch_ctl + 1;
    p.rays_launch = reinterpret_cast<unsigned long long*>(p.launch_ctl + 2);
  }
  return AMBER_OK;
}

int StartPixelMasks(amber_hip_pt* h, float* timing) {
  const uint32_t n_pixels = static_cast<uint32_t>(BandPixels(h));
  if (!(h->two_phase && h->env.pixel_mask) || n_pixels == 0 || (h->pixel_mask_ready && !timing)) return AMBER_OK;
  if (!h->d_pixel_mask) HIP_TRY(h->d_pixel_mask.alloc(n_pixels));
  PixelMaskArgs pm{};
  for (int i = 0; i < 4; i++) for (int c = 0; c < 3; c++) pm.ap[i][c] = static_cast<double>(h->aperture_rect[i][c]) - static_cast<double>(h->scene.fp_center[c]);
  pm.inv_w = 1.0 / static_cast<double>(h->scene.sensor.wf); pm.inv_h = 1.0 / static_cast<double>(h->scene.sensor.hf);
  pm.focal_scale = h->lens.kind == 1u ? -(8.0 * static_cast<double>(h->scene.fp_reach) + 1.0) / static_cast<double>(h->lens.sensor_distance)
                                      : static_cast<double>(h->lens.focus_distance) / -static_cast<double>(h->lens.sensor_distance);
  pm.row_begin = h->row_begin; pm.stripe_rows = h->stripe_rows; pm.stripe_period = h->stripe_period; pm.n_pixels = n_pixels;
  pm.block = (h->stripe_rows == 0u || h->stripe_rows % 4u == 0u) ? 4u : 1u;
  if (h->env.pixel_mask_block && (h->stripe_rows == 0u || h->stripe_rows % h->env.pixel_mask_block == 0u)) pm.block = h->env.pixel_mask_block;
  pm.local_rows = h->local_rows;
  pm.blocks_x = (h->scene.sensor.w + pm.block - 1u) / pm.block;
  pm.n_blocks = pm.blocks_x * ((h->local_rows + pm.block - 1u) / pm.block);
  {
    const DevScene& sc = h->scene;
    const double cx = sc.fp_center[0], cy = sc.fp_center[1], cz = sc.fp_center[2], reach = sc.fp_reach;
    const double world_mag = std::max(std::max(std::fabs(cx), std::max(std::fabs(cy), std::fabs(cz))) + reach,
                                      std::max(std::fabs(double(h->lens.origin[0])), std::max(std::fabs(double(h->lens.origin[1])), std::fabs(double(h->lens.origin[2])))));
    const double slack = 1e-5 * reach + 32.0 * 5.9604644775390625e-08 * world_mag;
    pm.planes_cut_a = h->host_planes.size() > 32 ? 0xffffffffu : 0u;
    for (size_t i = 0; i < h->host_planes.size() && i < 32; i++) {
      const DevPlane& q = h->host_planes[i];
      bool above = true, below = true;
      for (int k = 0; k < 4; k++) {
        const double sa = double(q.n[0]) * pm.ap[k][0] + double(q.n[1]) * pm.ap[k][1] + double(q.n[2]) * pm.ap[k][2] - double(q.d0);
        above = above && sa > 10.0 * slack; below = below && sa < -10.0 * slack;
      }
      if (!(above || below)) pm.planes_cut_a |= 1u << i;
    }
  }
  Event ev0, ev1;
  if (timing) { HIP_TRY(hipEventCreate(&ev0.v)); HIP_TRY(hipEventCreate(&ev1.v)); HIP_TRY(hipEventRecord(ev0.v, h->stream)); }
  hipLaunchKernelGGL(pixel_mask_kernel, dim3((pm.n_blocks + 15u) / 16u), dim3(256), 0, h->stream, h->scene, pm, h->d_pixel_mask);
  HIP_TRY(hipGetLastError());
  if (timing) { HIP_TRY(hipEventRecord(ev1.v, h->stream)); HIP_TRY(hipEventSynchronize(ev1.v)); HIP_TRY(hipEventElapsedTime(timing, ev0.v, ev1.v)); }
  h->pixel_mask_ready = true;
  return AMBER_OK;
}

template <bool kSig>
int LaunchPathKernel(const amber_hip_pt* h, bool pool, uint32_t n_blocks, const RenderArgs& a) {
  return WithHitEngine(h->hit_engine, [&](auto engine) -> int {
    constexpr int kEngine = decltype(engine)::value;
#ifdef AMBER_LAB
    if (kEngine == ENGINE_BVH && pool) { hipLaunchKernelGGL((pt_bvh_pool_kernel<kSig>), dim3(n_blocks), dim3(256), 0, h->stream, a); return AMBER_OK; }
#endif
    hipLaunchKernelGGL((pt_megakernel<kEngine, false, kSig>), dim3(n_blocks), dim3(256), 0, h->stream, a);
    return AMBER_OK;
  });
}


int BeginPathLaunch(amber_hip_pt* h, uint32_t n, uint32_t n_pixels, bool sig) {
  PathLaunchBufs& p = h->paths;
  const uint64_t n_paths = static_cast<uint64_t>(n_pixels) * n;
  const size_t need_words = static_cast<size_t>((n_paths + 31u) / 32u) + 4u;
  if (need_words > p.flags.n) {
    AMBER_TRY(Grow(h, p.flags, need_words, "path bitmap"));
    p.flags_dirty = true;
  }
  const size_t touched_words = static_cast<size_t>(n_pixels) / 32u + 2u;
  AMBER_TRY(Grow(h, p.touched, touched_words, "touched pixels"));
  AMBER_TRY(Grow(h, p.excl, n_pixels, "pixel ranks"));
  AMBER_TRY(Grow(h, p.block_sum, static_cast<size_t>(n_pixels) / 256u + 2u, "pixel ranks"));
  AMBER_TRY(EnsureLaunchCtl(h));
  if (!p.h_rec_count.v) HIP_TRY(hipHostMalloc(reinterpret_cast<void**>(&p.h_rec_count.v), sizeof(unsigned int), hipHostMallocDefault));
  if (!p.pending_event.v) HIP_TRY(hipEventCreateWithFlags(&p.pending_event.v, hipEventDisableTiming));
  HIP_TRY(hipMemsetAsync(p.launch_ctl, 0, 4 * sizeof(unsigned int), h->stream));
  if (p.flags_dirty) HIP_TRY(hipMemsetAsync(p.flags, 0, p.flags.n * sizeof(uint32_t), h->stream));
  p.flags_dirty = sig || (n & 31u) != 0u;
  HIP_TRY(hipMemsetAsync(p.touched, 0, touched_words * sizeof(uint32_t), h->stream));
  return AMBER_OK;
}

void SetRecordArgs(const amber_hip_pt* h, RenderArgs& a) {
  const PathLaunchBufs& p = h->paths;
  a.flags = p.flags; a.touched = p.touched; a.records = p.records; a.rec_count = p.rec_count; a.rec_capacity = p.rec_capacity;
  a.ray_count = p.rays_launch; a.next_item = p.launch_ctl;
}

int FinishPathLaunch(amber_hip_pt* h, uint32_t first, uint32_t n, uint32_t n_pixels, float* target, const RecordProducer& producer, bool cannot_run_out) {
  PathLaunchBufs& p = h->paths;
  const uint32_t n_rank_blocks = (n_pixels + 255u) / 256u;
  hipLaunchKernelGGL(rec_rank_kernel, dim3(n_rank_blocks), dim3(256), 0, h->stream, p.flags, p.touched, n_pixels, n, p.excl, p.block_sum);
  hipLaunchKernelGGL(rec_scan_blocks_kernel, dim3(1), dim3(1024), 0, h->stream, p.block_sum, n_rank_blocks, p.rec_count, p.rec_capacity, h->d_rays, p.rays_launch);
  hipLaunchKernelGGL(rec_place_kernel, dim3(static_cast<uint32_t>(h->n_cus) * 8u), dim3(256), 0, h->stream, p.records, p.rec_count, p.rec_capacity, p.flags,
                     p.excl, p.block_sum, n, MakeExactDiv(n), p.sorted);
  hipLaunchKernelGGL(reduce_flagged_kernel, dim3(n_rank_blocks), dim3(256), 0, h->stream, target, p.flags, p.touched, p.sorted, p.excl, p.block_sum,
                     p.rec_count, p.rec_capacity, n_pixels, n);
  HIP_TRY(hipGetLastError());
  HIP_TRY(hipMemcpyAsync(p.h_rec_count.v, p.rec_count, sizeof(unsigned int), hipMemcpyDeviceToHost, h->stream));
  HIP_TRY(hipEventRecord(p.pending_event.v, h->stream));
  p.pending = true; p.pending_first = first; p.pending_n = n; p.pending_target = target; p.pending_producer = producer;
  p.pending_checked = cannot_run_out;
  ++p.n_launches;
  return AMBER_OK;
}

int LaunchPaths(amber_hip_pt* h, uint32_t first, uint32_t n, uint32_t n_pixels, float* target, unsigned long long* sig) {
  PathLaunchBufs& p = h->paths;
  const uint64_t n_paths = static_cast<uint64_t>(n_pixels) * n;
#ifdef AMBER_LAB
  const bool bvh = h->hit_engine == AMBER_ENGINE_BVH && !h->bvh_paths;
#else
  const bool bvh = false;
  if (sig) return Fail(AMBER_EINVAL, "path signatures are part of the lab build");
#endif
  const uint32_t n_blocks = PersistentBlocks(h, n_paths, bvh);
  AMBER_TRY(CheckRefStack(h, n_blocks));
  {
    size_t carried = static_cast<size_t>(PersistentBlocks(h)) * 256u * 3u * 2u;
#ifdef AMBER_LAB
    if (bvh) carried = static_cast<size_t>(h->n_cus) * AMBER_BVH_POOL_WGS * 4u * AMBER_BVH_POOL_CARRIED_PER_WAVE;
#endif
    AMBER_TRY(Grow(h, p.carried, carried, "carried measurements"));
  }
#ifdef AMBER_LAB
  if (bvh) AMBER_TRY(Grow(h, h->d_bvh_stack, static_cast<size_t>(h->n_cus) * AMBER_BVH_POOL_WGS * 256u * AMBER_BVH_POOL_GLOBAL_LEVELS, "traversal stacks"));
#endif
  AMBER_TRY(BeginPathLaunch(h, n, n_pixels, sig != nullptr));
  RenderArgs a = MakeRenderArgs(h, h->hashed_seed, n_pixels, first, n);
  a.pixel_mask = h->pixel_mask_ready ? h->d_pixel_mask : nullptr;
  SetRecordArgs(h, a);
  a.stamps = h->d_stamps;
  a.bvh_stack = h->d_bvh_stack; a.carried = p.carried; a.sig = sig; a.n_items = static_cast<uint32_t>(n_paths);
  AMBER_TRY(TimedLaunch(h, true, [&]() -> int {
#ifdef AMBER_LAB
    if (sig) return LaunchPathKernel<true>(h, bvh, n_blocks, a);
#endif
    return LaunchPathKernel<false>(h, bvh, n_blocks, a);
  }));
  if (sig) return AMBER_OK;
  return FinishPathLaunch(h, first, n, n_pixels, target, RecordProducer{}, n_paths + RecordSlack(h) <= p.rec_capacity);
}

#ifdef AMBER_LAB
int LaunchLabRecords(amber_hip_pt* h, uint32_t n, uint32_t n_pixels, float* target, const RecordProducer& producer);
#endif

int ResolvePending(amber_hip_pt* h) {
  PathLaunchBufs& p = h->paths;
  while (p.pending) {
    HIP_TRY(hipEventSynchronize(p.pending_event.v));
    p.pending = false;
    const uint64_t used = *p.h_rec_count.v;
    const uint64_t n_paths = BandPixels(h) * p.pending_n;
    p.rec_density = n_paths ? static_cast<double>(used) / static_cast<double>(n_paths) : 0.0;
    p.density_known = true;
    if (used <= p.rec_capacity) break;
    p.flags_dirty = true;
    ++p.n_repeats;
    AMBER_TRY(EnsureRecordCapacity(h, used + used / 4u + RecordSlack(h)));
#ifdef AMBER_LAB
    if (p.pending_producer.lab) {
      const RecordProducer producer = p.pending_producer;
      AMBER_TRY(LaunchLabRecords(h, p.pending_n, static_cast<uint32_t>(BandPixels(h)), p.pending_target, producer));
      continue;
    }
#endif
    AMBER_TRY(LaunchPaths(h, p.pending_first, p.pending_n, static_cast<uint32_t>(BandPixels(h)), p.pending_target, nullptr));
  }
  return AMBER_OK;
}

int SettlePending(amber_hip_pt* h) { return h->paths.pending && !h->paths.pending_checked ? ResolvePending(h) : AMBER_OK; }

int RenderPassPaths(amber_hip_pt* h, uint32_t first_sample, uint32_t n_samples, uint32_t n_pixels, float* target, unsigned long long* sig) {
  PathLaunchBufs& p = h->paths;
  if (sig) {
    AMBER_TRY(EnsureRecordCapacity(h, RecordSlack(h)));
    return LaunchPaths(h, first_sample, n_samples, n_pixels, target, sig);
  }
  const uint64_t slack = h->env.test_density_scale > 0 ? 64u : RecordSlack(h);
  return SplitSamples(first_sample, n_samples, "band too large for one launch", [&](uint32_t left, amber_plan::Launch* l) -> int {
    if (p.pending && (!p.pending_checked || !p.density_known)) AMBER_TRY(ResolvePending(h));
    *l = amber_plan::PathLaunch(n_pixels, left, p.density_known, p.rec_density, h->env.test_density_scale, slack);
    return AMBER_OK;
  }, [&](uint32_t first, const amber_plan::Launch& l, bool*) -> int {
    if (l.slots > p.rec_capacity) {
      if (p.pending) AMBER_TRY(ResolvePending(h));
      AMBER_TRY(EnsureRecordCapacity(h, l.slots));
    }
    return LaunchPaths(h, first, l.n, n_pixels, target, nullptr);
  });
}

int RenderPassBvhItems(amber_hip_pt* h, uint32_t first_sample, uint32_t n_samples, uint32_t n_pixels, float* target, unsigned long long* sig) {
#ifndef AMBER_LAB
  if (sig) return Fail(AMBER_EINVAL, "path signatures are part of the lab build");
#endif
  return SplitSamples(first_sample, n_samples, "band too large for one launch", [&](uint32_t left, amber_plan::Launch* l) -> int {
    *l = amber_plan::ItemLaunch(n_pixels, left);
    return AMBER_OK;
  }, [&](uint32_t first, const amber_plan::Launch& l, bool*) -> int {
    const uint32_t n_chunks = (l.n + AMBER_ACCUM_CHUNK - 1) / AMBER_ACCUM_CHUNK;
    AMBER_TRY(Grow(h, h->d_partial, static_cast<size_t>(n_chunks) * n_pixels * 3u, "partial sums"));
    if (sig && l.n != n_samples) return Fail(AMBER_EINVAL, "too many paths for one signature launch");
    if (sig) AMBER_TRY(EnsureLaunchCtl(h));
    RenderArgs a = MakeRenderArgs(h, h->hashed_seed, n_pixels, first, l.n);
    a.partial = h->d_partial; a.ray_count = sig ? h->paths.rays_launch : h->d_rays; a.next_item = h->d_next; a.stamps = h->d_stamps;
    a.n_items = n_pixels * n_chunks; a.sig = sig; a.shade_batch = h->bvh_shade_batch;
    const uint32_t n_blocks = PersistentBlocks(h, a.n_items);
    HIP_TRY(hipMemsetAsync(h->d_next, 0, sizeof(unsigned int), h->stream));
    AMBER_TRY(TimedLaunch(h, true, [&]() -> int {
#ifdef AMBER_LAB
      if (sig) { hipLaunchKernelGGL((pt_bvh_megakernel<false, 24, true>), dim3(n_blocks), dim3(256), 0, h->stream, a); return AMBER_OK; }
#endif
      hipLaunchKernelGGL((pt_bvh_megakernel<false, 24>), dim3(n_blocks), dim3(256), 0, h->stream, a);
      return AMBER_OK;
    }));
    if (sig) return AMBER_OK;
    const uint32_t n_elems = n_pixels * 3u;
    hipLaunchKernelGGL(reduce_partials_kernel, dim3((n_elems + 255u) / 256u), dim3(256), 0, h->stream, target, h->d_partial, n_elems, n_chunks);
    HIP_TRY(hipGetLastError());
    return AMBER_OK;
// ... 61 lines not shown
```

### amber_amd/csrc/hip/pt_megakernel.inc

```

#define AMBER_WAVE_TIME_SLOTS 8192u
#ifndef AMBER_MEGAKERNEL_WAVES_PER_SIMD
#define AMBER_MEGAKERNEL_WAVES_PER_SIMD 6
#endif
#ifndef AMBER_CLAIM_PATHS
#define AMBER_CLAIM_PATHS 1024u
#endif
template <bool kLight> struct PoolLayout { static constexpr int kChunks = 4; };

#ifndef AMBER_PATH_BVH_STACK
#define AMBER_PATH_BVH_STACK 12
#endif
#define AMBER_KERNEL_PHOTONS 0x100
template <int kEngineSink, bool kLight = false, bool kSig = false>
__global__ void __launch_bounds__(256, (kEngineSink & ~AMBER_KERNEL_PHOTONS) == ENGINE_BVH ? 5 : AMBER_MEGAKERNEL_WAVES_PER_SIMD) pt_megakernel(const RenderArgs a) {
  constexpr int kEngine = kEngineSink & ~AMBER_KERNEL_PHOTONS;
  constexpr bool kPhotons = (kEngineSink & AMBER_KERNEL_PHOTONS) != 0;
  static_assert(kLight || !kPhotons, "vertices are recorded along light paths");
  const DevScene& sc = a.scene;
  const uint32_t lane = threadIdx.x & 63u;
  constexpr bool kTwoPhase = EngineTraits<kEngine>::kTwoPhase;
  constexpr int kChunks = PoolLayout<kLight>::kChunks;
  constexpr bool kCold = !kLight && kEngine != ENGINE_BVH;
  constexpr bool kDivBasis = kCold && (AMBER_SHARED_DIV_NORMALIZE & 1), kDivHit = kCold && (AMBER_SHARED_DIV_NORMALIZE & 2), kDivEye = kCold && (AMBER_SHARED_DIV_NORMALIZE & 4);
  constexpr uint32_t kSqrtMask = kCold ? static_cast<uint32_t>(AMBER_EXACT_SQRT) : 0u;
#define AMBER_ARG(cold, field) (kCold ? AMBER_COLD(cold, field) : a.field)
#define AMBER_COLD_OPEN() (kCold ? ColdArgs::Open() : ColdArgs{nullptr})
  __shared__ uint4 lds_pool[4][64 * kChunks];
  const EngineLds lds = StageEngineLds<kEngine, AMBER_PATH_BVH_STACK>(sc);
  const uint32_t wave_in_block = __builtin_amdgcn_readfirstlane(threadIdx.x >> 6);
  uint4* pool = lds_pool[wave_in_block];

  uint32_t claim_next = 0, claim_end = 0;
  uint32_t pool_count = 0;
  uint32_t rec_next = 0, rec_end = 0;
  bool exhausted = false;
  bool retired = false, alive = false;
  uint32_t q = 0;
  bool carries = false;
  auto block_index = []() -> size_t { uint32_t b = blockIdx.x; if (kCold) asm volatile("" : "+s"(b)); return b; };
  auto carried_slot = [&]() -> float* {
    const uint32_t t = wave_in_block * 64u + BvhStackHybrid::LaneId();
    return AMBER_ARG(AMBER_COLD_OPEN(), carried) + (block_index() * 256u + t) * 3u;
  };
#define AMBER_CARRIED() carried_slot()
  auto carried_parked = [&](uint32_t pool_slot) -> float* {
    return AMBER_ARG(AMBER_COLD_OPEN(), carried) + (static_cast<size_t>(gridDim.x) * 256u + (block_index() * 4u + wave_in_block) * 64u + pool_slot) * 3u;
  };
  V3 o = v3(0.f, 0.f, 0.f), d = v3(0.f, 0.f, 1.f), w = v3(0.f, 0.f, 0.f);
  uint64_t rng = 1;
  uint32_t casts = 0;
  uint32_t rays_wave = 0;
  int origin_slot = -1;
  uint32_t sig_obj = 2166136261u, sig_t = 2166136261u;
#ifdef AMBER_STAMPS
  StampCtx stamp_store{}; StampCtx* stamp_ctx = &stamp_store;
  stamp_ctx->last = __builtin_amdgcn_s_memtime();
  unsigned long long* wave_times = a.stamps ? a.stamps + 8 + 4ull * ((blockIdx.x * 4u + wave_in_block) % AMBER_WAVE_TIME_SLOTS) : nullptr;
  if (wave_times && lane == 0) { wave_times[0] = wall_clock64(); wave_times[1] = 0; wave_times[2] = 0; }
#endif

  for (;;) {
    AMBER_STAMP(6);
    const bool need = !alive && !retired;
    const unsigned long long mask = __ballot(need);
    bool primary = false;
    uint32_t premask = 0u;
    if (mask) {
      const uint32_t n_need = static_cast<uint32_t>(__popcll(mask));
      const uint32_t rank = __builtin_amdgcn_mbcnt_hi(static_cast<uint32_t>(mask >> 32), __builtin_amdgcn_mbcnt_lo(static_cast<uint32_t>(mask), 0u));
      const uint32_t take = pool_count < n_need ? pool_count : n_need;
      if (need && rank < take) {
        const uint32_t sl = pool_count - 1u - rank;
        const uint4 c0 = pool[sl * kChunks + 0], c1 = pool[sl * kChunks + 1], c2 = pool[sl * kChunks + 2], c3 = pool[sl * kChunks + 3];
        o = v3(__uint_as_float(c0.x), __uint_as_float(c0.y), __uint_as_float(c0.z));
        d = v3(__uint_as_float(c0.w), __uint_as_float(c1.x), __uint_as_float(c1.y));
        w = v3(__uint_as_float(c1.z), __uint_as_float(c1.w), __uint_as_float(c2.x));
        rng = static_cast<uint64_t>(c2.y) | (static_cast<uint64_t>(c2.z) << 32);
        q = c2.w;
        casts = c3.x & 0x7fffffffu; carries = (c3.x >> 31) != 0u;
        if (!kLight && carries) { const float* from = carried_parked(sl); float* to = AMBER_CARRIED(); to[0] = from[0]; to[1] = from[1]; to[2] = from[2]; }
        origin_slot = static_cast<int>(c3.y);
        if (kSig) { sig_obj = c3.z; sig_t = c3.w; }
        alive = true;
      }
      __builtin_amdgcn_wave_barrier();
      pool_count -= take;
      if (take < n_need && !exhausted) {
        AMBER_STAMP(0);
        if (claim_next == claim_end) {
          const ColdArgs cold = AMBER_COLD_OPEN();
          const uint32_t size = AMBER_CLAIM_PATHS;
          uint32_t base = 0;
          const uint32_t n_items = AMBER_ARG(cold, n_items);
          if (lane == 0) base = atomicAdd(AMBER_ARG(cold, next_item), size);
          base = __builtin_amdgcn_readfirstlane(base);
          if (base >= n_items) exhausted = true;
          else { claim_next = base; claim_end = n_items - base < size ? n_items : base + size; }
#ifdef AMBER_STAMPS
          if (wave_times && lane == 0) { if (exhausted) wave_times[2] = wall_clock64(); else if (wave_times[1] == 0) wave_times[1] = wall_clock64(); }
#endif
        }
        if (!exhausted) {
          const uint32_t n_new = claim_end - claim_next < 64u ? claim_end - claim_next : 64u;
          const uint32_t gbase = claim_next;
          claim_next += n_new;
          const unsigned long long m_alive = __ballot(alive);
          if (alive) {
            const uint32_t sl = __builtin_amdgcn_mbcnt_hi(static_cast<uint32_t>(m_alive >> 32), __builtin_amdgcn_mbcnt_lo(static_cast<uint32_t>(m_alive), 0u));
            pool[sl * kChunks + 0] = make_uint4(__float_as_uint(o.x), __float_as_uint(o.y), __float_as_uint(o.z), __float_as_uint(d.x));
            pool[sl * kChunks + 1] = make_uint4(__float_as_uint(d.y), __float_as_uint(d.z), __float_as_uint(w.x), __float_as_uint(w.y));
            pool[sl * kChunks + 2] = make_uint4(__float_as_uint(w.z), static_cast<uint32_t>(rng), static_cast<uint32_t>(rng >> 32), q);
            pool[sl * kChunks + 3] = make_uint4(casts | (carries ? 0x80000000u : 0u), static_cast<uint32_t>(origin_slot), sig_obj, sig_t);
            if (!kLight && carries) { const float* from = AMBER_CARRIED(); float* to = carried_parked(sl); to[0] = from[0]; to[1] = from[1]; to[2] = from[2]; }
          }
          pool_count = static_cast<uint32_t>(__popcll(m_alive));
          __builtin_amdgcn_wave_barrier();
          alive = lane < n_new;
          const ColdArgs cold = AMBER_COLD_OPEN();
          if (alive) {
            q = gbase + lane;
            const uint32_t n_samples = AMBER_ARG(cold, n_samples), first_sample = AMBER_ARG(cold, first_sample);
            const uint32_t plocal = Quotient(AMBER_ARG(cold, div_samples), q), sample = first_sample + (q - plocal * n_samples);
            if (kLight) {
              rng = XorShiftSeed(a.hashed_seed, a.path_offset + plocal, sample);
              GenerateLightRay(sc, rng, o, d, w, origin_slot);
            } else {
              const uint32_t lrow = Quotient(AMBER_ARG(cold, div_width), plocal);
              const EyeRayScene eye{AMBER_ARG(cold, scene.lens), AMBER_ARG(cold, scene.blades), AMBER_ARG(cold, scene.sensor)};
              const uint32_t row_begin = AMBER_ARG(cold, row_begin), stripe_rows = AMBER_ARG(cold, stripe_rows);
              const uint32_t px = plocal - lrow * eye.sensor.w;
              uint32_t py = row_begin + lrow;
              if (stripe_rows) {
                const uint32_t band = Quotient(AMBER_ARG(cold, div_stripe_rows), lrow);
                py = row_begin + band * AMBER_ARG(cold, stripe_period) + (lrow - band * stripe_rows);
              }
              rng = XorShiftSeed(AMBER_ARG(cold, hashed_seed), px + py * eye.sensor.w, sample);
              float ew;
              bool near_edge = false;
              GenerateEyeRay<kDivEye, SqrtModeOf(kSqrtMask, 4u)>(eye, px, py, rng, o, d, ew, origin_slot, &near_edge);
              w = v3(ew, ew, ew);
              const uint32_t* const pixel_mask = kTwoPhase ? AMBER_ARG(cold, pixel_mask) : nullptr;
              if (kTwoPhase && pixel_mask) {
                premask = pixel_mask[plocal] | (origin_slot >= 0 ? 1u << origin_slot : 0u) | (near_edge ? AMBER_ARG(cold, scene.blade_mask) : 0u);
              }
            }
            carries = false;
            casts = 0;
            if (kSig) { sig_obj = 2166136261u; sig_t = 2166136261u; }
          }
          primary = kTwoPhase && !kLight && AMBER_ARG(AMBER_COLD_OPEN(), pixel_mask) != nullptr;
          AMBER_STAMP(1);
        }
      }
      if (!alive && !retired && pool_count == 0u && exhausted) retired = true;
      if (__ballot(!retired) == 0ull) break;
    }

    rays_wave += static_cast<uint32_t>(__popcll(__ballot(alive)));
    bool emit = false;
    V3 meas = v3(0.f, 0.f, 0.f);
    if (alive) {
      if (!kLight && carries) meas = ld3(AMBER_CARRIED());
      if (kLight) {
        const uint32_t plocal = Quotient(a.div_samples, q);
        const typename std::conditional<kPhotons, PhotonSink, SplatSink>::type sink = MakeLightSink<kPhotons>(a, a.path_offset + plocal, a.first_sample + (q - plocal * a.n_samples));
        alive = PathStep<false, kEngine, true, false, false, 0u, kPhotons ? SINK_PHOTONS : SINK_SPLATS>(sc, lds.objects, lds.stack, o, d, w, meas, rng, casts, origin_slot, nullptr AMBER_STAMP_ARG, &sink, false, 0u, AMBER_PATH_BVH_STACK);
      } else if (kSig) {
        Bounce b;
        alive = PathStep<true, kEngine, false, kDivBasis, kDivHit, kSqrtMask>(sc, lds.objects, lds.stack, o, d, w, meas, rng, casts, origin_slot, &b AMBER_STAMP_ARG, nullptr, primary, premask, AMBER_PATH_BVH_STACK);
        sig_obj = Fnv32(sig_obj, static_cast<uint32_t>(b.object));
        if (b.object >= 0) sig_t = Fnv32(sig_t, __float_as_uint(b.t));
        if (!alive) AMBER_ARG(AMBER_COLD_OPEN(), sig)[q] = static_cast<unsigned long long>(sig_obj) | (static_cast<unsigned long long>(sig_t) << 32);
      } else {
        alive = PathStep<false, kEngine, false, kDivBasis, kDivHit, kSqrtMask>(sc, lds.objects, lds.stack, o, d, w, meas, rng, casts, origin_slot, nullptr AMBER_STAMP_ARG, nullptr, primary, premask, AMBER_PATH_BVH_STACK);
      }
      if (!kLight) {
        const bool nz = (__float_as_uint(meas.x) | __float_as_uint(meas.y) | __float_as_uint(meas.z)) != 0u;
        emit = !alive && nz;
        if (alive && nz) { float* c = AMBER_CARRIED(); c[0] = meas.x; c[1] = meas.y; c[2] = meas.z; carries = true; }
      }
    }
    if (!kLight && !kCold) EmitRecords(a, emit, q, meas, rec_next, rec_end);
    if (kCold) {
      EmitRecords([]() {
        const ColdArgs cold = ColdArgs::Open();
        return RecordSink{AMBER_COLD(cold, records), AMBER_COLD(cold, flags), AMBER_COLD(cold, touched), AMBER_COLD(cold, rec_count), AMBER_COLD(cold, rec_capacity), AMBER_COLD(cold, div_samples)};
      }, emit, q, meas, rec_next, rec_end);
    }
  }

#undef AMBER_COLD_OPEN
#undef AMBER_ARG
#undef AMBER_CARRIED
  if (!kLight) CloseRecords(a, rec_next, rec_end);
#ifdef AMBER_STAMPS
  if (lane == 0 && a.stamps) for (int k = 0; k < 8; k++) atomicAdd(a.stamps + k, stamp_ctx->acc[k]);
  if (wave_times && lane == 0) wave_times[3] = wall_clock64();
#endif
  if (lane == 0 && rays_wave) atomicAdd(a.ray_count, static_cast<unsigned long long>(rays_wave));
}
```

### amber_amd/csrc/hip/scene_prep.h

```cpp
#pragma once

#include <algorithm>
#include <chrono>
#include <cmath>
#include <cstdio>
#include <cstdlib>
#include <cstring>
#include <string>
#include <vector>

#include "../../../include/amber_hip.h"
#include "bvh_build.h"
#include "filter_build.h"
#include "ref_bvh_build.h"

namespace amber_prep {

using namespace amber_dev;

constexpr uint32_t kHitTwoPhaseN = 5;
constexpr uint32_t kTwoPhaseAutoObjects = 80;

struct EnvSwitches {
  uint32_t two_phase_auto = kTwoPhaseAutoObjects;
  int bvh_pool = -1;
  uint32_t bvh_shade_batch = 0;
  bool bvh_paths_off = false;
  uint32_t bvh_paths_max_depth = 0xffffffffu;
  bool debug_bvh = false, debug_filter = false;
  bool pixel_mask = true;
  uint32_t pixel_mask_block = 0;
  double test_density_scale = 0;
  uint32_t test_device_build_max_depth = 0;
};

inline EnvSwitches ReadEnv() {
  EnvSwitches e;
  const char* ev;
  if ((ev = std::getenv("AMBER_TWO_PHASE_MAX_OBJECTS")) && std::atoi(ev) >= 0) e.two_phase_auto = std::min<uint32_t>(AMBER_MAX_GROUP_OBJECTS, static_cast<uint32_t>(std::atoi(ev)));
#ifdef AMBER_LAB
  if ((ev = std::getenv("AMBER_BVH_POOL")) && (ev[0] == '0' || ev[0] == '1')) e.bvh_pool = ev[0] == '1';
#endif
  if ((ev = std::getenv("AMBER_BVH_SHADE_BATCH")) && std::atoi(ev) >= 1 && std::atoi(ev) <= 64) e.bvh_shade_batch = static_cast<uint32_t>(std::atoi(ev));
  e.bvh_paths_off = (ev = std::getenv("AMBER_BVH_PATHS")) && ev[0] == '0';
  if ((ev = std::getenv("AMBER_BVH_PATHS_MAX_DEPTH"))) e.bvh_paths_max_depth = static_cast<uint32_t>(std::atoi(ev));
  e.debug_bvh = std::getenv("AMBER_DEBUG_BVH") != nullptr;
  e.debug_filter = std::getenv("AMBER_DEBUG_FILTER") != nullptr;
  e.pixel_mask = !((ev = std::getenv("AMBER_PIXEL_MASK")) && ev[0] == '0');
  if ((ev = std::getenv("AMBER_PIXEL_MASK_BLOCK")) && (ev[0] == '1' || ev[0] == '2' || ev[0] == '4') && ev[1] == 0) e.pixel_mask_block = static_cast<uint32_t>(ev[0] - '0');
  if ((ev = std::getenv("AMBER_TEST_RECORD_DENSITY_SCALE"))) e.test_density_scale = std::atof(ev);
  if ((ev = std::getenv("AMBER_TEST_DEVICE_BUILD_MAX_DEPTH")) && std::atoi(ev) > 0) e.test_device_build_max_depth = static_cast<uint32_t>(std::atoi(ev));
  return e;
}

struct SceneState {
  uint32_t engine = AMBER_ENGINE_LIST;
  uint32_t hit_engine = AMBER_ENGINE_LIST;
  bool two_phase = false;
  bool bvh_pool = false;
  bool bvh_paths = false;
  uint32_t bvh_shade_batch = 0;
  DevScene scene{};
  DevLens lens{};
  float aperture_rect[4][3] = {};
  std::vector<uint32_t> prog_order;
  std::vector<DevPlane> host_planes;
  AmberBuildInfo build{};
};

inline void ChooseBvhScheduler(SceneState& st, size_t n_objects, size_t n_triangles, uint32_t flags, const EnvSwitches& env,
                               size_t n_nodes, uint32_t depth, uint32_t path_bvh_stack, uint32_t shade_batch) {
  st.bvh_paths = !st.bvh_pool && !(flags & AMBER_PT_FLAG_BVH_ITEMS) && st.engine != AMBER_ENGINE_WAVEFRONT && depth <= path_bvh_stack;
  st.bvh_shade_batch = 2u * n_triangles > n_objects ? 40u : shade_batch;
  if (env.bvh_shade_batch) st.bvh_shade_batch = env.bvh_shade_batch;
  if (env.bvh_paths_off || env.bvh_paths_max_depth < depth) st.bvh_paths = false;
  if (env.debug_bvh) std::fprintf(stderr, "amber_hip: BVH of %zu objects: %zu nodes, depth %u; scheduler %s, shading batch %u\n", n_objects, n_nodes, depth,
                                  st.bvh_pool ? "pt_bvh_pool_kernel" : (st.bvh_paths ? "pt_megakernel<ENGINE_BVH>" : "pt_bvh_megakernel"), st.bvh_shade_batch);
}
inline size_t CountTriangles(const std::vector<DevObject>& objs) {
  size_t n_triangles = 0;
  for (const DevObject& ob : objs) n_triangles += (ob.kind & 0xffu) == AMBER_PRIM_TRIANGLE ? 1u : 0u;
  return n_triangles;
}
inline void ChooseBvhScheduler(SceneState& st, const std::vector<DevObject>& objs, const AmberPtParams* params, const EnvSwitches& env,
                               size_t n_nodes, uint32_t depth, uint32_t path_bvh_stack, uint32_t shade_batch) {
  ChooseBvhScheduler(st, objs.size(), CountTriangles(objs), params->reserved, env, n_nodes, depth, path_bvh_stack, shade_batch);
}

inline amber_bvh::FlatBvh BuildHostTree(SceneState& st, const std::vector<DevObject>& objs, const AmberPtParams* params, const EnvSwitches& env,
                                        uint32_t path_bvh_stack, uint32_t shade_batch) {
  const auto t0 = std::chrono::steady_clock::now();
  amber_bvh::FlatBvh bvh = amber_bvh::BuildBvh(objs);
  st.build.tree_ms += std::chrono::duration<double, std::milli>(std::chrono::steady_clock::now() - t0).count();
  if (env.debug_bvh) {
    const amber_bvh::BvhQuality q = amber_bvh::MeasureBvh(bvh.nodes, bvh.root_ref);
    std::fprintf(stderr, "amber_hip: BVH %s: SAH inner-node term %.3f, leaf term %.3f (x objects %.3f), leaf volume / scene volume %.3f; %u inner nodes, %u leaves, %u levels\n",
                 "as built", q.inner_area, q.leaf_area, q.leaf_object_area, q.leaf_volume, q.inner, q.leaves, q.depth);
  }
  ChooseBvhScheduler(st, objs, params, env, bvh.nodes.size(), bvh.depth, path_bvh_stack, shade_batch);
  st.build.where = st.build.fallback_reason ? AMBER_BUILD_HOST_FALLBACK : AMBER_BUILD_HOST;
  st.build.n_nodes = static_cast<uint32_t>(bvh.nodes.size()); st.build.n_leaves = st.build.n_nodes + 1u; st.build.depth = bvh.depth;
  return bvh;
}

inline void SetBvhRayMargin(DevScene& sc, const float bounds_min[3], const float bounds_max[3], bool has_spheres, float min_sphere_radius) {
  double d2 = 0;
  for (int c = 0; c < 3; c++) {
    sc.bvh_center[c] = 0.5f * (bounds_min[c] + bounds_max[c]);
    const double e = double(bounds_max[c]) - bounds_min[c];
    d2 += e * e;
  }
  sc.bvh_half_diag = static_cast<float>(0.5 * std::sqrt(d2) * 1.0001);
  sc.bvh_inv_rmin = !has_spheres ? 0.0f : (min_sphere_radius > 0 ? static_cast<float>(std::min(3.0e38, 1.0001 / min_sphere_radius)) : 3.0e38f);
}


inline void DeriveLens(const AmberFlatThinLens& L, const AmberFlatObject* blade_records, const AmberSensor& sensor, const float fp_center[3], float fp_reach,
                       DevLens& lens, std::vector<DevBlade>& blades, float aperture_rect[4][3]) {
  blades.resize(L.n_blades);
  for (uint32_t i = 0; i < L.n_blades; i++) {
    const AmberFlatObject& f = blade_records[i];
    for (int c = 0; c < 3; c++) { blades[i].v0[c] = f.p[c]; blades[i].v1[c] = f.p[3 + c]; blades[i].v2[c] = f.p[6 + c]; blades[i].n[c] = f.p[9 + c]; }
    blades[i].slot = -1; blades[i].pad[0] = blades[i].pad[1] = blades[i].pad[2] = 0;
  }
  {
    double lo[2] = {1e300, 1e300}, hi[2] = {-1e300, -1e300};
    for (const DevBlade& bl : blades)
      for (const float* v : {bl.v0, bl.v1, bl.v2}) {
        const double r[3] = {double(v[0]) - L.origin[0], double(v[1]) - L.origin[1], double(v[2]) - L.origin[2]};
        for (int c = 0; c < 2; c++) {
          const double x = L.local_[3 * c] * r[0] + L.local_[3 * c + 1] * r[1] + L.local_[3 * c + 2] * r[2];
          lo[c] = std::min(lo[c], x); hi[c] = std::max(hi[c], x);
        }
      }
    double world_mag = 0;
    for (int c = 0; c < 3; c++) world_mag = std::max({world_mag, std::fabs(double(fp_center[c])) + fp_reach, std::fabs(double(L.origin[c]))});
    for (int c = 0; c < 2; c++) { const double m = 1e-3 * (hi[c] - lo[c]) + 1e-6 + 1e-5 * fp_reach + 32.0 * 5.9604644775390625e-08 * world_mag; lo[c] -= m; hi[c] += m; }
    for (int i = 0; i < 4; i++) {
      const double x = (i & 1) ? hi[0] : lo[0], y = (i & 2) ? hi[1] : lo[1];
      for (int c = 0; c < 3; c++) aperture_rect[i][c] = static_cast<float>(L.origin[c] + (L.kind == AMBER_LENS_PINHOLE ? 0.0 : L.global_[3 * c] * x + L.global_[3 * c + 1] * y));
    }
  }
  std::memset(&lens, 0, sizeof lens);
  std::memcpy(lens.origin, L.origin, sizeof L.origin);
  std::memcpy(lens.global_, L.global_, sizeof L.global_);
  std::memcpy(lens.local_, L.local_, sizeof L.local_);
  lens.focus_distance = L.focus_distance; lens.sensor_distance = L.sensor_distance; lens.p_area = L.p_area;
  { volatile float q = -L.focus_distance / L.sensor_distance; lens.neg_fd_over_sd = q; }
  {
    volatile float size_f = static_cast<float>(static_cast<uint64_t>(sensor.width) * sensor.height);
    volatile float area = sensor.scene_width * sensor.scene_height;
    volatile float r = size_f / area;
    lens.size_over_area = r;
  }
  lens.sd2 = static_cast<double>(L.sensor_distance) * static_cast<double>(L.sensor_distance);
  lens.n_blades = L.n_blades; lens.n_blades_f = static_cast<float>(L.n_blades);
  lens.kind = L.kind;
  { volatile float area = sensor.scene_width * sensor.scene_height; volatile float inv = 1.0f / area; lens.inv_scene_area = inv; }
  { volatile float q = -L.sensor_distance / L.focus_distance; lens.neg_sd_over_fd = q; }
  {
    double world_mag = 0, min_edge = 1e300;
    for (int c = 0; c < 3; c++) world_mag = std::max(world_mag, std::fabs(double(L.origin[c])));
    for (const DevBlade& bl : blades) {
      const float* v[3] = {bl.v0, bl.v1, bl.v2};
      for (int k = 0; k < 3; k++) {
        double e2 = 0;
        for (int c = 0; c < 3; c++) { const double e = double(v[k][c]) - v[(k + 1) % 3][c]; e2 += e * e; world_mag = std::max(world_mag, std::fabs(double(v[k][c]))); }
        min_edge = std::min(min_edge, std::sqrt(e2));
      }
    }
    const double tol = min_edge > 0 ? std::max(1e-3, 64.0 * 5.9604644775390625e-08 * world_mag / min_edge) : 1.0;
    lens.edge_tol = static_cast<float>(std::min(1.0, tol));
  }
}

inline void DeriveLensOfState(const SceneState& st, const AmberFlatThinLens& L, const AmberFlatObject* blade_records,
                              DevLens& lens, std::vector<DevBlade>& blades, float aperture_rect[4][3]) {
  const AmberSensor sensor{st.scene.sensor.w, st.scene.sensor.h, st.scene.sensor.sw, st.scene.sensor.sh};
  DeriveLens(L, blade_records, sensor, st.scene.fp_center, st.scene.fp_reach, lens, blades, aperture_rect);
}

struct PreparedScene : SceneState {
  std::string error;
  bool bvh_pending = false;
  uint32_t ref_depth = 0;
  std::vector<DevObject> objects;
  std::vector<DevMaterial> materials;
  std::vector<DevBlade> blades;
  std::vector<DevPlane> planes;
  std::vector<DevTriFilter> tri_filters;
  std::vector<DevSphereFilter> sphere_filters;
  std::vector<DevObject> prog_objects;
  std::vector<DevFilterGroup> groups;
  std::vector<DevLight> lights;
  std::vector<DevBvhNodeQ> bvh_nodes;
  std::vector<DevBvhNodeQ4> bvh_nodes4;
  std::vector<uint32_t> bvh_prims;
  std::vector<DevObject> bvh_objects;
  std::vector<float4> bvh_spheres, bvh_tris;
  std::vector<DevRefNode> ref_nodes;
  std::vector<DevRefLeaf> ref_leaves;
};

inline void FillBvhArrays(SceneState& st, PreparedScene& p, const std::vector<DevObject>& objs, amber_bvh::FlatBvh& bvh) {
  const auto t0 = std::chrono::steady_clock::now();
  amber_bvh::QuantizedBvh qbvh = amber_bvh::QuantizeBvh(bvh.nodes, bvh.root_ref, [&](uint32_t slot) { return objs[bvh.prim_index[slot]].kind & 0xffu; });
#if AMBER_BVH_WIDE
  {
    amber_bvh::QuantizedBvh4 q4 = amber_bvh::CollapseBvh4(bvh.nodes, bvh.root_ref, qbvh, [&](uint32_t slot) { return objs[bvh.prim_index[slot]].kind & 0xffu; });
    p.bvh_nodes4 = std::move(q4.nodes);
    qbvh.root_ref = q4.root_ref;
  }
#endif
  p.bvh_nodes = std::move(qbvh.nodes);
  {
    std::vector<DevObject>& leaf_order = p.bvh_objects;
    std::vector<float4>& leaf_spheres = p.bvh_spheres;
    leaf_order.resize(bvh.prim_index.size());
    leaf_spheres.resize(bvh.prim_index.size());
    for (size_t k = 0; k < leaf_order.size(); k++) {
      const DevObject& ob = objs[bvh.prim_index[k]];
      leaf_order[k] = ob;
      leaf_spheres[k] = (ob.kind & 0xffu) == AMBER_PRIM_SPHERE ? make_float4(ob.a[0], ob.a[1], ob.a[2], ob.radius) : make_float4(0.f, 0.f, 0.f, 0.f);
    }
    bool any_tri = false;
    for (const DevObject& ob : leaf_order) any_tri = any_tri || (ob.kind & 0xffu) == AMBER_PRIM_TRIANGLE;
    std::vector<float4>& leaf_tris = p.bvh_tris;
    leaf_tris.resize(any_tri ? 3 * leaf_order.size() : 0);
    for (size_t k = 0; any_tri && k < leaf_order.size(); k++) {
      const DevObject& ob = leaf_order[k];
      if ((ob.kind & 0xffu) != AMBER_PRIM_TRIANGLE) { leaf_tris[3 * k] = leaf_tris[3 * k + 1] = leaf_tris[3 * k + 2] = make_float4(0.f, 0.f, 0.f, 0.f); continue; }
      float idx; const uint32_t scene_index = bvh.prim_index[k]; std::memcpy(&idx, &scene_index, 4);
      leaf_tris[3 * k] = make_float4(ob.a[0], ob.a[1], ob.a[2], ob.e1[0]);
      leaf_tris[3 * k + 1] = make_float4(ob.e1[1], ob.e1[2], ob.e2[0], ob.e2[1]);
      leaf_tris[3 * k + 2] = make_float4(ob.e2[2], idx, 0.f, 0.f);
    }
  }
  p.bvh_prims = std::move(bvh.prim_index);
  DevScene& sc = st.scene;
  sc.bvh_root = qbvh.root_ref;
  for (int c = 0; c < 3; c++) { sc.bvh_gmin[c] = qbvh.gmin[c]; sc.bvh_step[c] = qbvh.step[c]; sc.bvh_reach[c] = qbvh.reach[c]; }
  SetBvhRayMargin(sc, bvh.bounds_min, bvh.bounds_max, bvh.has_spheres, bvh.min_sphere_radius);
  if (st.hit_engine == AMBER_ENGINE_BVH) st.build.tree_ms += std::chrono::duration<double, std::milli>(std::chrono::steady_clock::now() - t0).count();
}

inline void HostBvhFallback(SceneState& st, PreparedScene& p, uint32_t reason, const AmberPtParams* params, const EnvSwitches& env, uint32_t path_bvh_stack, uint32_t shade_batch) {
  st.build.fallback_reason = reason;
  amber_bvh::FlatBvh bvh = BuildHostTree(st, p.objects, params, env, path_bvh_stack, shade_batch);
  FillBvhArrays(st, p, p.objects, bvh);
  p.bvh_pending = false;
}

inline PreparedScene PrepareScene(const AmberFlatScene* s, const AmberSensor* sensor, const AmberPtParams* params, const EnvSwitches& env,
                                  uint32_t path_bvh_stack, uint32_t shade_batch) {
  PreparedScene p;
  p.bvh_shade_batch = shade_batch;
// ... 167 lines not shown
```

### include/amber_hip.h

```cpp
#ifndef AMBER_HIP_H
#define AMBER_HIP_H

#include <stdint.h>

#ifdef __cplusplus
extern "C" {
#endif
#pragma GCC visibility push(default)

#define AMBER_HIP_ABI_VERSION 3

#define AMBER_ACCUM_CHUNK 8u

enum {
  AMBER_OK = 0,
  AMBER_EINVAL = -1,
  AMBER_ENODEVICE = -2,
  AMBER_EHIP = -3,
  AMBER_ENOMEM = -4
};

enum { AMBER_PRIM_TRIANGLE = 0, AMBER_PRIM_SPHERE = 1, AMBER_PRIM_DISK = 2, AMBER_PRIM_CYLINDER = 3 };
enum {
  AMBER_MAT_LAMBERTIAN = 0,
  AMBER_MAT_PHONG = 1,
  AMBER_MAT_SPECULAR = 2,
  AMBER_MAT_REFRACTION = 3,
  AMBER_MAT_DIFFUSE_LIGHT = 4,
  AMBER_MAT_EYE = 5
};

typedef struct {
  uint32_t kind;
  uint32_t material;
  float    p[12];
} AmberFlatObject;

typedef struct {
  uint32_t kind;
  float    rho[3];
  float    param;
  float    r0;
} AmberFlatMaterial;

enum { AMBER_LENS_THIN = 0, AMBER_LENS_PINHOLE = 1 };
typedef struct {
  float    origin[3];
  float    global_[9];
  float    local_[9];
  float    focus_distance;
  float    sensor_distance;
  float    p_area;
  uint32_t n_blades;
  uint32_t first_blade_object;
  uint32_t kind;
} AmberFlatThinLens;

typedef struct {
  uint32_t object;
  float    cum_power;
  float    pdf_area;
  float    irradiance[3];
} AmberFlatLight;

typedef struct {
  const AmberFlatObject*   objects;
  uint32_t                 n_objects;
  const AmberFlatMaterial* materials;
  uint32_t                 n_materials;
  AmberFlatThinLens        lens;
  const AmberFlatLight*    lights;
  uint32_t                 n_lights;
} AmberFlatScene;

typedef struct {
  uint32_t width, height;
  float    scene_width, scene_height;
} AmberSensor;

typedef struct {
  uint64_t seed;
  uint32_t max_depth;
  int32_t  device;
  uint32_t row_begin;
  uint32_t row_end;
  void*    stream;
  uint32_t engine;
  uint32_t stripe_rows;
  uint32_t stripe_period;
  uint32_t reserved;
} AmberPtParams;
enum {
  AMBER_PT_FLAG_NULL_STREAM = 1u,
  AMBER_PT_FLAG_BVH_POOL = 2u,
  AMBER_PT_FLAG_BVH_ITEMS = 4u,
  AMBER_PT_FLAG_DEVICE_BUILD = 8u
};

enum {
  AMBER_ENGINE_AUTO = 0,
  AMBER_ENGINE_LIST = 1,
  AMBER_ENGINE_TWO_PHASE = 2,
  AMBER_ENGINE_BVH = 3,
  AMBER_ENGINE_WAVEFRONT = 4,
  AMBER_ENGINE_REFERENCE_BVH = 6
};

#pragma GCC visibility push(hidden)
typedef struct amber_hip_pt amber_hip_pt;
#pragma GCC visibility pop

int  amber_hip_pt_create(const AmberFlatScene* scene, const AmberSensor* sensor,
                         const AmberPtParams* params, amber_hip_pt** out);
int  amber_hip_pt_render_pass(amber_hip_pt*, uint32_t first_sample, uint32_t n_samples);
int  amber_hip_pt_clear(amber_hip_pt*);
int  amber_hip_pt_sync(amber_hip_pt*);
int  amber_hip_pt_download(amber_hip_pt*, float* rgb_sum, uint64_t* ray_count);
int  amber_hip_pt_device_framebuffer(amber_hip_pt*, void** dptr, uint64_t* n_floats);
int  amber_hip_pt_stream(amber_hip_pt*, void** stream);
int  amber_hip_pt_local_rows(amber_hip_pt*, uint32_t* n_rows);
enum { AMBER_BUILD_NONE = 0,
       AMBER_BUILD_HOST = 1, AMBER_BUILD_DEVICE = 2,
       AMBER_BUILD_HOST_FALLBACK = 3 };
enum { AMBER_BUILD_REASON_NONE = 0,
       AMBER_BUILD_REASON_DEPTH = 1,
       AMBER_BUILD_REASON_WIDE = 2,
       AMBER_BUILD_REASON_BOUNDS = 3 };
typedef struct {
  uint32_t where;
  uint32_t fallback_reason;
  uint32_t n_nodes;
  uint32_t n_leaves;
  uint32_t depth;
  uint32_t pad;
  double   tree_ms;
  double   create_ms;
} AmberBuildInfo;
int  amber_hip_pt_build_info(amber_hip_pt*, AmberBuildInfo* out);
enum { AMBER_UPDATE_REFIT = 0, AMBER_UPDATE_REBUILD = 1 };
typedef struct {
  uint32_t mode_used;
  uint32_t fallback_reason;
  uint32_t n_nodes, depth;
  float    area_before, area_after;
  double   update_ms;
} AmberUpdateInfo;
int  amber_hip_pt_update_objects(amber_hip_pt*, uint32_t first, uint32_t count, const AmberFlatObject* objects, uint32_t mode,
                                 AmberUpdateInfo* info );
int  amber_hip_pt_update_lens(amber_hip_pt*, const AmberFlatThinLens* lens, const AmberFlatObject* blades ,
                              uint32_t mode , AmberUpdateInfo* info );
typedef struct { float origin[3]; float t_max; float dir[3]; uint32_t pad; } AmberRay;
typedef struct { float t; int32_t object; float pos[3]; float normal[3]; } AmberRayHit;
enum { AMBER_RAYS_HOST = 1u };
int  amber_hip_pt_cast_rays(amber_hip_pt*, uint64_t n, const AmberRay* rays, AmberRayHit* hits, uint32_t flags);
int  amber_hip_pt_occluded(amber_hip_pt*, uint64_t n, const AmberRay* rays, uint8_t* occluded, uint32_t flags);
typedef struct { float origin[3]; uint32_t pad0; float dir[3]; uint32_t pad1;
                 float weight[3]; uint32_t pad2; uint64_t rng_state; uint64_t pad3; } AmberPathRay;
typedef struct { float rgb[3]; uint32_t casts; uint64_t rng_state; uint32_t pad[2]; } AmberPathResult;
int  amber_hip_pt_trace_paths(amber_hip_pt*, uint64_t n, const AmberPathRay* rays, AmberPathResult* out,
                              uint32_t n_samples, uint32_t max_depth , uint32_t flags );
uint64_t amber_hip_sampler_state(uint64_t seed, uint32_t pixel, uint32_t sample);
enum { AMBER_RESOLVE_MEAN_F32 = 0, AMBER_RESOLVE_RGB8 = 1, AMBER_RESOLVE_RGBA8 = 2 };
enum { AMBER_RESOLVE_HOST = 1u, AMBER_RESOLVE_MIRROR_X = 2u };
int  amber_hip_pt_resolve(amber_hip_pt*, uint32_t n_samples, uint32_t format, void* out, uint64_t out_bytes, uint32_t flags);
typedef struct { float albedo[3]; float depth; float normal[3]; float coverage; } AmberAovPixel;
int  amber_hip_pt_aov_pass(amber_hip_pt*, uint32_t first_sample, uint32_t n_samples);
int  amber_hip_pt_aov_clear(amber_hip_pt*);
int  amber_hip_pt_aov_download(amber_hip_pt*, AmberAovPixel* out);
int  amber_hip_pt_device_aov(amber_hip_pt*, void** dptr, uint64_t* n_pixels);
typedef struct { uint32_t levels; float k_normal; float k_albedo; float k_depth; float k_color; uint32_t reserved[3]; } AmberDenoiseParams;
int  amber_hip_pt_denoise(amber_hip_pt*, uint32_t n_samples, const AmberDenoiseParams* params,
                          uint32_t format, void* out, uint64_t out_bytes, uint32_t flags);
typedef struct { float m1, m2, batches, pad; } AmberMomentsPixel;
int  amber_hip_pt_render_batch(amber_hip_pt*, uint32_t first_sample, uint32_t n_samples);
int  amber_hip_pt_moments_clear(amber_hip_pt*);
int  amber_hip_pt_moments_download(amber_hip_pt*, AmberMomentsPixel* out);
int  amber_hip_pt_device_moments(amber_hip_pt*, void** dptr, uint64_t* n_pixels);
typedef struct { uint32_t levels; float k_normal; float k_albedo; float k_depth; float k_lum; uint32_t var_radius; uint32_t reserved[2]; } AmberDenoiseVarianceParams;
int  amber_hip_pt_denoise_variance(amber_hip_pt*, uint32_t n_samples, const AmberDenoiseVarianceParams* params,
// ... 50 lines not shown
```

### include/amber_hip_lab.h

```cpp
#ifndef AMBER_HIP_LAB_H
#define AMBER_HIP_LAB_H

#include "amber_hip.h"

#ifdef __cplusplus
extern "C" {
#endif
#pragma GCC visibility push(default)

int amber_hip_kat_cast(amber_hip_pt*, uint32_t n, const float* origins , const float* dirs ,
                       int32_t* out_object, float* out_t, float* out_pos , float* out_normal );
int amber_hip_kat_phase_a(amber_hip_pt*, uint32_t n, const float* origins , const float* dirs , int axis_loops,
                          uint32_t* out_mask, uint64_t mask_capacity, uint32_t* out_n_groups);
int amber_hip_kat_sample(amber_hip_pt*, uint32_t n, const uint32_t* material , const float* normals,
                         const float* dirs_out, uint64_t* rng_state , float* out_dir_in, float* out_weight);
int amber_hip_kat_eye(amber_hip_pt*, uint32_t n, const uint32_t* pixel, const uint32_t* sample, float* out7);
int amber_hip_kat_light_ray(amber_hip_pt*, uint32_t n, uint64_t* rng_state , float* out_origin , float* out_dir ,
                            float* out_weight , uint32_t* out_light );
int amber_hip_kat_lens_response(amber_hip_pt*, uint32_t n, const float* position , const float* direction_out ,
                                uint32_t* out_reached , uint32_t* out_pixel , float* out_value );
int amber_hip_kat_radiance(amber_hip_pt*, uint32_t n, const uint32_t* material , const float* normals , const float* dirs_out ,
                           float* out );
struct amber_host_scene;
int amber_host_kat_scene_lights(const struct amber_host_scene*, AmberFlatLight* lights, uint32_t* n_lights);
int amber_hip_kat_trace(amber_hip_pt*, uint32_t n, const uint32_t* pixel, const uint32_t* sample,
                        uint32_t max_bounces, uint32_t* out_records , uint32_t* out_casts );
int amber_hip_kat_signatures(amber_hip_pt*, uint32_t first_sample, uint32_t n_samples, uint64_t* out);
int amber_hip_pt_signatures(amber_hip_pt*, uint32_t first_sample, uint32_t n_samples, uint64_t* out);
int amber_hip_kat_traversal_rate(amber_hip_pt*, uint32_t n, const float* origins, const float* dirs, uint32_t waves, uint32_t refill_min,
                                 uint32_t repeats, float* out_t, int32_t* out_object, double* best_ms, uint32_t* out_rounds);
int amber_hip_kat_pixel_masks(amber_hip_pt*, uint32_t* out_mask, uint32_t* out_slot_of_object, uint32_t* out_always_mask, double* kernel_ms);
typedef struct { uint32_t n_nodes, n_prims; int32_t root; uint32_t depth; float gmin[3], step[3], reach[3]; } AmberBvhDump;
int amber_hip_kat_bvh_dump(amber_hip_pt*, uint32_t* nodes, uint32_t node_capacity, uint32_t* prims, uint32_t prim_capacity, AmberBvhDump* info);
int amber_hip_kat_lt_accumulate(amber_hip_pt*, const AmberSplat* records , uint32_t n);
typedef struct { uint32_t n_launches, n_repeats, rec_count, flag_words_set, flags_dirty; } AmberAccumulateInfo;
int amber_hip_kat_accumulate(amber_hip_pt*, uint32_t n_samples, const uint32_t* q , const float* rgb , uint32_t n_items,
                             uint32_t n_waves, uint32_t rec_capacity, uint64_t rays, AmberAccumulateInfo* info);
int amber_hip_kat_lt_stage_ms(amber_hip_pt*, double* sort_ms, double* sum_ms);
int amber_hip_kat_photon_stage_ms(amber_hip_pt*, double* trace_ms, double* sort_ms, double* gather_ms);
int amber_hip_kat_math(int device, int mode, uint32_t n, const float* x, float* out);
int amber_hip_kat_division(int device, int mode, uint32_t n, const float* x, float* out);
int amber_hip_kat_sqrt(int device, int mode, uint32_t n, const float* x, float* out);
typedef struct { uint64_t mismatches, in_range; uint32_t n_offenders, offenders[8]; int32_t seed_low, seed_high; } AmberSqrtSweep;
int amber_hip_kat_sqrt_sweep(int device, uint32_t first_bits, uint64_t count, AmberSqrtSweep* out);

#pragma GCC visibility pop
#ifdef __cplusplus
}
#endif
#endif
```

Baseline: 48090.

## Add scout megakernel pass that bounds path weights and replays suspect paths exactly

Adds a scout variant of the two-phase megakernel that traces paths with cheaper eye-ray weights and an integer log2 bound on path throughput, instead of computing the full weight per bounce. Paths whose bound is exceeded are written as records and recomputed exactly by a new replay kernel. The scout is enabled by default when the lens and materials pass host-side sanity checks. It aims to cut per-bounce weight arithmetic and register pressure in the common case, but adds a second kernel launch and duplicated tracing for flagged paths.

```diff
diff --git a/amber_amd/api.py b/amber_amd/api.py
--- a/amber_amd/api.py
+++ b/amber_amd/api.py
@@ -157,6 +157,7 @@
 ENGINE_REFERENCE_BVH = 6
 PT_FLAG_NULL_STREAM, PT_FLAG_BVH_POOL, PT_FLAG_BVH_ITEMS = 1, 2, 4
 PT_FLAG_DEVICE_BUILD = 8
+PT_FLAG_NO_SCOUT = 16
 BUILD_NONE, BUILD_HOST, BUILD_DEVICE, BUILD_HOST_FALLBACK = 0, 1, 2, 3
 BUILD_REASON_NONE, BUILD_REASON_DEPTH, BUILD_REASON_WIDE, BUILD_REASON_BOUNDS = 0, 1, 2, 3
 RAYS_HOST = 1
@@ -188,7 +189,7 @@
     "amber_hip_kat_sqrt", "amber_hip_kat_sqrt_sweep", "amber_hip_kat_lt_accumulate", "amber_hip_kat_lt_stage_ms",
     "amber_hip_kat_photon_stage_ms",
     "amber_hip_kat_light_ray", "amber_hip_kat_lens_response", "amber_hip_kat_radiance", "amber_host_kat_scene_lights",
-    "amber_hip_kat_accumulate", "amber_hip_kat_phase_a",
+    "amber_hip_kat_accumulate", "amber_hip_kat_phase_a", "amber_hip_kat_scout_flags",
 ]
 PRODUCT_LIB, LAB_LIB = "libamber_hip.so", "libamber_hip_lab.so"
 
@@ -299,6 +300,8 @@
             lib.amber_hip_kat_lens_response.argtypes = [vp, u32, vp, vp, vp, vp, vp]
             lib.amber_hip_kat_radiance.argtypes = [vp, u32, vp, vp, vp, vp]
             lib.amber_host_kat_scene_lights.argtypes = [vp, C.POINTER(FlatLight), C.POINTER(u32)]
+        if hasattr(lib, "amber_hip_kat_scout_flags"):
+            lib.amber_hip_kat_scout_flags.argtypes = [vp, u32, u32, vp, u64, C.POINTER(u32), C.POINTER(u32)]
         if hasattr(lib, "amber_hip_kat_accumulate"):
             lib.amber_hip_kat_accumulate.argtypes = [vp, u32, vp, vp, u32, u32, u32, u64, C.POINTER(AccumulateInfo)]
     lib.amber_host_cornell_box.restype = vp
@@ -825,6 +828,14 @@
                                                        len(qq), n_waves, rec_capacity, rays, C.byref(info)))
         return {k: int(getattr(info, k)) for k, _ in AccumulateInfo._fields_}
 
+    def kat_scout_flags(self, first_sample: int, n_samples: int):
+        n_paths = len(self.row_index) * self.sensor.width * n_samples
+        words = np.zeros((n_paths + 31) // 32 + 1, np.uint32)
+        scouts, bound0 = C.c_uint32(), C.c_uint32()
+        _check(load_library().amber_hip_kat_scout_flags(self._h, first_sample, n_samples, words.ctypes.data, len(words), C.byref(scouts), C.byref(bound0)))
+        self.scout_bound0 = int(bound0.value)
+        return np.unpackbits(words.view(np.uint8), bitorder="little")[:n_paths].astype(bool), bool(scouts.value)
+
     def kat_lt_stage_ms(self):
         a, b = C.c_double(), C.c_double()
         _check(load_library().amber_hip_kat_lt_stage_ms(self._h, C.byref(a), C.byref(b)))
diff --git a/amber_amd/csrc/hip/dev_shading.h b/amber_amd/csrc/hip/dev_shading.h
--- a/amber_amd/csrc/hip/dev_shading.h
+++ b/amber_amd/csrc/hip/dev_shading.h
@@ -193,7 +193,7 @@
 }
 
 struct EyeRayScene { const DevLens* lens; const DevBlade* blades; DevSensor sensor; };
-template <bool kSharedDiv = false, int kSqrt = SQRT_PLAIN, typename Scene>
+template <bool kSharedDiv = false, int kSqrt = SQRT_PLAIN, bool kScout = false, typename Scene>
 __device__ __forceinline__ void GenerateEyeRay(const Scene& sc, uint32_t px, uint32_t py, uint64_t& rng,
                                                V3& origin, V3& dir, float& weight, int& origin_slot, bool* near_edge = nullptr) {
   const DevLens L = LoadLens(sc.lens);
@@ -204,12 +204,16 @@
     const float uvy = (static_cast<float>(py) + jy) / sc.sensor.hf;
     const V3 sensor_point = v3((uvx - 0.5f) * sc.sensor.sw, (uvy - 0.5f) * sc.sensor.sh, L.sensor_distance);
     const V3 ray_dir = Normalize<kSharedDiv, kSqrt>(MatMul(L.global_, -sensor_point));
-    const V3 dl = MatMul(L.local_, ray_dir);
-    const V3 point = (L.sensor_distance / dl.z) * dl;
-    const float geometry_factor = dl.z * dl.z / SquaredLength(point);
-    const float pdf_dir = L.inv_scene_area / geometry_factor;
     origin = ld3(L.origin); dir = ray_dir;
-    weight = 1.0f / 1.0f / pdf_dir;
+    if (kScout) {
+      weight = L.local_[6] * ray_dir.x + L.local_[7] * ray_dir.y + L.local_[8] * ray_dir.z;
+    } else {
+      const V3 dl = MatMul(L.local_, ray_dir);
+      const V3 point = (L.sensor_distance / dl.z) * dl;
+      const float geometry_factor = dl.z * dl.z / SquaredLength(point);
+      const float pdf_dir = L.inv_scene_area / geometry_factor;
+      weight = 1.0f / 1.0f / pdf_dir;
+    }
     origin_slot = -1;
     if (near_edge) *near_edge = true;
     return;
@@ -230,6 +234,13 @@
   const float uvy = (static_cast<float>(py) + jy) / sc.sensor.hf;
   const V3 sensor_point = v3((uvx - 0.5f) * sc.sensor.sw, (uvy - 0.5f) * sc.sensor.sh, L.sensor_distance);
   const V3 direction = Normalize<kSharedDiv, kSqrt>(L.neg_fd_over_sd * sensor_point - aperture_point);
+  if (kScout) {
+    origin = ap_origin; dir = Normalize<kSharedDiv, kSqrt>(MatMul(L.global_, direction));
+    origin_slot = bl->slot;
+    const bool sound = IsFinite(direction.x) && IsFinite(direction.y) && Abs(L.sensor_distance - aperture_point.z) >= amber_scout::kMinGap;
+    weight = sound ? direction.z : __builtin_nanf("");
+    return;
+  }
   const double factor = Pow4(Normalize<false, kSqrt>(sensor_point - aperture_point).z / direction.z);
   const V3 ray_dir = Normalize<kSharedDiv, kSqrt>(MatMul(L.global_, direction));
   const V3 dloc = MatMul(L.local_, ray_dir);
@@ -243,7 +254,7 @@
 
 struct SplatSink { DevSplat* records; unsigned int* count; uint32_t capacity; uint32_t path, sample; float size_f; };
 
-enum { SINK_SPLATS = 0, SINK_PHOTONS = 1 };
+enum { SINK_SPLATS = 0, SINK_PHOTONS = 1, SINK_SCOUT = 2 };
 struct PhotonSink : SplatSink { float4* photons; uint32_t surfaces; };
 #ifndef AMBER_PHOTON_CLAIM_PER_LANE
 #define AMBER_PHOTON_CLAIM_PER_LANE 0
@@ -251,20 +262,21 @@
 
 template <bool kTrace, int kEngine, bool kLight, bool kDivBasis = false, bool kDivHit = false, uint32_t kSqrtMask = 0u, int kSink = SINK_SPLATS>
 __device__ __forceinline__ bool PathShade(const DevScene& sc, const DevObject* lds_objects, const HitRec& h, V3& o, V3& d, V3& weight, V3& measurement,
-                                          uint64_t& rng, uint32_t& casts, int& origin_slot, Bounce* trace AMBER_STAMP_PARAM, const SplatSink* sink);
+                                          uint64_t& rng, uint32_t& casts, int& origin_slot, Bounce* trace AMBER_STAMP_PARAM, const SplatSink* sink, uint32_t* scout_bound = nullptr);
 
 template <bool kTrace, int kEngine, bool kLight = false, bool kDivBasis = false, bool kDivHit = false, uint32_t kSqrtMask = 0u, int kSink = SINK_SPLATS>
 __device__ __forceinline__ bool PathStep(const DevScene& sc, const DevObject* lds_objects, int32_t* lds_stack, V3& o, V3& d, V3& weight, V3& measurement,
                                          uint64_t& rng, uint32_t& casts, int& origin_slot, Bounce* trace AMBER_STAMP_PARAM, const SplatSink* sink = nullptr,
-                                         const bool use_premask = false, const uint32_t premask = 0u, const int bvh_stack_cap = AMBER_BVH_STACK) {
+                                         const bool use_premask = false, const uint32_t premask = 0u, const int bvh_stack_cap = AMBER_BVH_STACK, uint32_t* scout_bound = nullptr) {
   HitRec h;
   ClosestHit<kEngine, (kSqrtMask & 8u) ? SQRT_EXACT : SQRT_PLAIN>(sc, lds_objects, lds_stack, o, d, origin_slot, h AMBER_STAMP_ARG, use_premask, premask, bvh_stack_cap);
-  return PathShade<kTrace, kEngine, kLight, kDivBasis, kDivHit, kSqrtMask, kSink>(sc, lds_objects, h, o, d, weight, measurement, rng, casts, origin_slot, trace AMBER_STAMP_ARG, sink);
+  return PathShade<kTrace, kEngine, kLight, kDivBasis, kDivHit, kSqrtMask, kSink>(sc, lds_objects, h, o, d, weight, measurement, rng, casts, origin_slot, trace AMBER_STAMP_ARG, sink, scout_bound);
 }
 
 template <bool kTrace, int kEngine, bool kLight, bool kDivBasis, bool kDivHit, uint32_t kSqrtMask, int kSink>
 __device__ __forceinline__ bool PathShade(const DevScene& sc, const DevObject* lds_objects, const HitRec& h, V3& o, V3& d, V3& weight, V3& measurement,
-                                          uint64_t& rng, uint32_t& casts, int& origin_slot, Bounce* trace AMBER_STAMP_PARAM, const SplatSink* splat_sink) {
+                                          uint64_t& rng, uint32_t& casts, int& origin_slot, Bounce* trace AMBER_STAMP_PARAM, const SplatSink* splat_sink, uint32_t* scout_bound) {
+  constexpr bool kScout = !kLight && kSink == SINK_SCOUT;
   casts++;
   if (h.idx < 0) {
     if (kTrace) { trace->object = -1; trace->t = __builtin_nanf(""); trace->pos = v3(0, 0, 0); trace->weight_before = v3(0, 0, 0); }
@@ -316,7 +328,8 @@
     AMBER_STAMP(4);
     SampleImportance(m, normal, dir_out, rng, dir_in, sw);
   } else {
-    measurement = measurement + weight * Radiance(m, normal, dir_out);
+    if (kScout) measurement = Radiance(m, normal, dir_out);
+    else measurement = measurement + weight * Radiance(m, normal, dir_out);
     AMBER_STAMP(4);
     SampleLight<kDivBasis, kSqrtMask>(m, normal, dir_out, rng, dir_in, sw);
   }
@@ -329,6 +342,10 @@
   o = pos; d = dir_in;
   if (kEngine == ENGINE_TWO_PHASE_N) origin_slot = (lds_objects[h.slot].kind & 0x80u) ? h.slot : -1;
   else origin_slot = (kEngine == ENGINE_TWO_PHASE && static_cast<uint32_t>(h.slot) < sc.n_prog_tris) ? h.slot : -1;
+  if (kScout) {
+    *scout_bound = amber_scout::BounceBound(*scout_bound, __float_as_uint(sw.x), __float_as_uint(sw.y), __float_as_uint(sw.z), __float_as_uint(p_rr));
+    return true;
+  }
 #if AMBER_SHARED_WEIGHT_QUOTIENT
   {
     const uint32_t bx = __float_as_uint(sw.x), by = __float_as_uint(sw.y), bz = __float_as_uint(sw.z);
diff --git a/amber_amd/csrc/hip/lab_api.inc b/amber_amd/csrc/hip/lab_api.inc
--- a/amber_amd/csrc/hip/lab_api.inc
+++ b/amber_amd/csrc/hip/lab_api.inc
@@ -455,6 +455,25 @@
   return AMBER_OK;
 }); }
 
+int amber_hip_kat_scout_flags(amber_hip_pt* h, uint32_t first_sample, uint32_t n_samples, uint32_t* out_flags, uint64_t n_words, uint32_t* out_scouts, uint32_t* out_bound0) {
+  return Guarded("amber_hip_kat_scout_flags", [&]() -> int {
+  if (!h || !out_flags) return Fail(AMBER_EINVAL, "null argument");
+  if (out_scouts) *out_scouts = h->scout ? 1u : 0u;
+  if (out_bound0) *out_bound0 = h->scout_bound0;
+  const uint64_t n_paths = BandPixels(h) * n_samples, need_words = (n_paths + 31u) / 32u;
+  if (n_samples == 0 || n_paths > kMaxPathsPerLaunch || static_cast<uint64_t>(first_sample) + n_samples > 0xffffffffull) return Fail(AMBER_EINVAL, "amber_hip_kat_scout_flags: no samples, or more paths than one launch takes");
+  if (n_words < need_words) return Fail(AMBER_EINVAL, "amber_hip_kat_scout_flags: the bitmap of this launch has " + std::to_string(need_words) + " words");
+  std::memset(out_flags, 0, n_words * sizeof(uint32_t));
+  if (!h->scout || n_paths == 0) return AMBER_OK;
+  HIP_TRY(hipSetDevice(h->device));
+  AMBER_TRY(ResolvePending(h));
+  AMBER_TRY(EnsureRecordCapacity(h, n_paths + RecordSlack(h)));
+  AMBER_TRY(LaunchPaths(h, first_sample, n_samples, static_cast<uint32_t>(BandPixels(h)), nullptr, nullptr, true));
+  HIP_TRY(hipMemcpyAsync(out_flags, h->paths.flags, need_words * sizeof(uint32_t), hipMemcpyDeviceToHost, h->stream));
+  HIP_TRY(hipStreamSynchronize(h->stream));
+  return AMBER_OK;
+}); }
+
 int amber_hip_kat_lt_stage_ms(amber_hip_pt* h, double* sort_ms, double* sum_ms) { return Guarded("amber_hip_kat_lt_stage_ms", [&]() -> int {
   if (!h) return Fail(AMBER_EINVAL, "null handle");
   h->lt.stage_timing = true;
diff --git a/amber_amd/csrc/hip/pt_args.h b/amber_amd/csrc/hip/pt_args.h
--- a/amber_amd/csrc/hip/pt_args.h
+++ b/amber_amd/csrc/hip/pt_args.h
@@ -8,6 +8,7 @@
   uint4* records;
   unsigned int* rec_count;
   uint32_t rec_capacity;
+  uint32_t scout_bound0;
   unsigned long long* ray_count;
   unsigned int* next_item;
   unsigned long long* stamps;
@@ -37,6 +38,8 @@
   }
   void SetSamples(uint32_t first_sample_, uint32_t n_samples_) { first_sample = first_sample_; n_samples = n_samples_; div_samples = MakeExactDiv(n_samples_); }
 };
+
+static_assert(offsetof(RenderArgs, scout_bound0) + 4 == offsetof(RenderArgs, ray_count), "scout_bound0 sits in what was padding");
 
 template <bool kPhotons>
 __device__ __forceinline__ typename std::conditional<kPhotons, PhotonSink, SplatSink>::type MakeLightSink(const RenderArgs& a, uint32_t path, uint32_t sample) {
diff --git a/amber_amd/csrc/hip/pt_device.h b/amber_amd/csrc/hip/pt_device.h
--- a/amber_amd/csrc/hip/pt_device.h
+++ b/amber_amd/csrc/hip/pt_device.h
@@ -11,4 +11,5 @@
 #include "dev_two_phase.h"
 #include "dev_bvh.h"
 #include "dev_closest_hit.h"
+#include "scout_bound.h"
 #include "dev_shading.h"
diff --git a/amber_amd/csrc/hip/pt_host.hip b/amber_amd/csrc/hip/pt_host.hip
--- a/amber_amd/csrc/hip/pt_host.hip
+++ b/amber_amd/csrc/hip/pt_host.hip
@@ -33,6 +33,7 @@
 #include "pt_args.h"
 #include "pt_megakernel.inc"
 #include "pt_records.inc"
+#include "pt_replay.inc"
 #include "pt_bvh_megakernel.inc"
 #ifdef AMBER_LAB
 #include "bvh_pool.inc"
@@ -216,6 +217,8 @@
   DevBuf<unsigned long long> d_sig;
   DevBuf<uint32_t> d_pixel_mask;
   bool pixel_mask_ready = false;
+  bool scout = false;
+  uint32_t scout_bound0 = 0;
   int n_cus = 256;
   uint32_t row_begin = 0, row_end = 0, stripe_rows = 0, stripe_period = 0, local_rows = 0;
   uint64_t seed = 0, hashed_seed = 0;
@@ -334,6 +337,9 @@
   DevScene& sc = h->scene;
   HIP_TRY(UploadTo(h->objects_buf, p.objects, 0, sc.objects));
   h->create_flags = params->reserved;
+#if AMBER_SCOUT
+  h->scout = amber_prep::DecideScout(h->engine, h->hit_engine, params->reserved, h->lens, p.blades, p.materials, sensor->scene_width, sensor->scene_height, &h->scout_bound0);
+#endif
   h->n_triangles = amber_prep::CountTriangles(p.objects);
   for (size_t i = 0; i < p.objects.size(); i++) {
     h->has_spheres = h->has_spheres || (p.objects[i].kind & 0xffu) == AMBER_PRIM_SPHERE;
diff --git a/amber_amd/csrc/hip/pt_launch.inc b/amber_amd/csrc/hip/pt_launch.inc
--- a/amber_amd/csrc/hip/pt_launch.inc
+++ b/amber_amd/csrc/hip/pt_launch.inc
@@ -169,6 +169,16 @@
   });
 }
 
+int LaunchScoutedPaths(const amber_hip_pt* h, uint32_t n_blocks, const RenderArgs& a, bool replay) {
+#if AMBER_SCOUT
+  hipLaunchKernelGGL((pt_megakernel<ENGINE_TWO_PHASE | AMBER_KERNEL_SCOUT>), dim3(n_blocks), dim3(256), 0, h->stream, a);
+  if (replay) hipLaunchKernelGGL((replay_records_kernel<ENGINE_TWO_PHASE>), dim3(static_cast<uint32_t>(h->n_cus) * 8u), dim3(256), 0, h->stream, a);
+  return AMBER_OK;
+#else
+  return Fail(AMBER_EINVAL, "this build has no scout (AMBER_SCOUT=0)");
+#endif
+}
+
 
 int BeginPathLaunch(amber_hip_pt* h, uint32_t n, uint32_t n_pixels, bool sig) {
   PathLaunchBufs& p = h->paths;
@@ -216,7 +226,7 @@
   return AMBER_OK;
 }
 
-int LaunchPaths(amber_hip_pt* h, uint32_t first, uint32_t n, uint32_t n_pixels, float* target, unsigned long long* sig) {
+int LaunchPaths(amber_hip_pt* h, uint32_t first, uint32_t n, uint32_t n_pixels, float* target, unsigned long long* sig, bool scout_only = false) {
   PathLaunchBufs& p = h->paths;
   const uint64_t n_paths = static_cast<uint64_t>(n_pixels) * n;
 #ifdef AMBER_LAB
@@ -237,19 +247,21 @@
 #ifdef AMBER_LAB
   if (bvh) AMBER_TRY(Grow(h, h->d_bvh_stack, static_cast<size_t>(h->n_cus) * AMBER_BVH_POOL_WGS * 256u * AMBER_BVH_POOL_GLOBAL_LEVELS, "traversal stacks"));
 #endif
-  AMBER_TRY(BeginPathLaunch(h, n, n_pixels, sig != nullptr));
+  AMBER_TRY(BeginPathLaunch(h, n, n_pixels, sig != nullptr || scout_only));
   RenderArgs a = MakeRenderArgs(h, h->hashed_seed, n_pixels, first, n);
+  a.scout_bound0 = h->scout_bound0;
   a.pixel_mask = h->pixel_mask_ready ? h->d_pixel_mask : nullptr;
   SetRecordArgs(h, a);
   a.stamps = h->d_stamps;
   a.bvh_stack = h->d_bvh_stack; a.carried = p.carried; a.sig = sig; a.n_items = static_cast<uint32_t>(n_paths);
-  AMBER_TRY(TimedLaunch(h, true, [&]() -> int {
+  AMBER_TRY(TimedLaunch(h, !scout_only, [&]() -> int {
 #ifdef AMBER_LAB
     if (sig) return LaunchPathKernel<true>(h, bvh, n_blocks, a);
 #endif
+    if (h->scout) return LaunchScoutedPaths(h, n_blocks, a, !scout_only);
     return LaunchPathKernel<false>(h, bvh, n_blocks, a);
   }));
-  if (sig) return AMBER_OK;
+  if (sig || scout_only) return AMBER_OK;
   return FinishPathLaunch(h, first, n, n_pixels, target, RecordProducer{}, n_paths + RecordSlack(h) <= p.rec_capacity);
 }
 
diff --git a/amber_amd/csrc/hip/pt_megakernel.inc b/amber_amd/csrc/hip/pt_megakernel.inc
--- a/amber_amd/csrc/hip/pt_megakernel.inc
+++ b/amber_amd/csrc/hip/pt_megakernel.inc
@@ -6,21 +6,27 @@
 #ifndef AMBER_CLAIM_PATHS
 #define AMBER_CLAIM_PATHS 1024u
 #endif
-template <bool kLight> struct PoolLayout { static constexpr int kChunks = 4; };
+template <bool kLight, bool kScout = false> struct PoolLayout { static constexpr int kChunks = kScout ? 3 : 4; };
 
 #ifndef AMBER_PATH_BVH_STACK
 #define AMBER_PATH_BVH_STACK 12
 #endif
 #define AMBER_KERNEL_PHOTONS 0x100
+#define AMBER_KERNEL_SCOUT 0x200
+#ifndef AMBER_SCOUT
+#define AMBER_SCOUT 1
+#endif
 template <int kEngineSink, bool kLight = false, bool kSig = false>
-__global__ void __launch_bounds__(256, (kEngineSink & ~AMBER_KERNEL_PHOTONS) == ENGINE_BVH ? 5 : AMBER_MEGAKERNEL_WAVES_PER_SIMD) pt_megakernel(const RenderArgs a) {
-  constexpr int kEngine = kEngineSink & ~AMBER_KERNEL_PHOTONS;
+__global__ void __launch_bounds__(256, (kEngineSink & ~(AMBER_KERNEL_PHOTONS | AMBER_KERNEL_SCOUT)) == ENGINE_BVH ? 5 : AMBER_MEGAKERNEL_WAVES_PER_SIMD) pt_megakernel(const RenderArgs a) {
+  constexpr int kEngine = kEngineSink & ~(AMBER_KERNEL_PHOTONS | AMBER_KERNEL_SCOUT);
   constexpr bool kPhotons = (kEngineSink & AMBER_KERNEL_PHOTONS) != 0;
+  constexpr bool kScout = (kEngineSink & AMBER_KERNEL_SCOUT) != 0;
   static_assert(kLight || !kPhotons, "vertices are recorded along light paths");
+  static_assert(!kScout || (kEngine == ENGINE_TWO_PHASE && !kLight && !kSig), "the scout is the headline kernel's loop");
   const DevScene& sc = a.scene;
   const uint32_t lane = threadIdx.x & 63u;
   constexpr bool kTwoPhase = EngineTraits<kEngine>::kTwoPhase;
-  constexpr int kChunks = PoolLayout<kLight>::kChunks;
+  constexpr int kChunks = PoolLayout<kLight, kScout>::kChunks;
   constexpr bool kCold = !kLight && kEngine != ENGINE_BVH;
   constexpr bool kDivBasis = kCold && (AMBER_SHARED_DIV_NORMALIZE & 1), kDivHit = kCold && (AMBER_SHARED_DIV_NORMALIZE & 2), kDivEye = kCold && (AMBER_SHARED_DIV_NORMALIZE & 4);
   constexpr uint32_t kSqrtMask = kCold ? static_cast<uint32_t>(AMBER_EXACT_SQRT) : 0u;
@@ -50,6 +56,7 @@
   V3 o = v3(0.f, 0.f, 0.f), d = v3(0.f, 0.f, 1.f), w = v3(0.f, 0.f, 0.f);
   uint64_t rng = 1;
   uint32_t casts = 0;
+  uint32_t scout_bound = 0;
   uint32_t rays_wave = 0;
   int origin_slot = -1;
   uint32_t sig_obj = 2166136261u, sig_t = 2166136261u;
@@ -70,7 +77,17 @@
       const uint32_t n_need = static_cast<uint32_t>(__popcll(mask));
       const uint32_t rank = __builtin_amdgcn_mbcnt_hi(static_cast<uint32_t>(mask >> 32), __builtin_amdgcn_mbcnt_lo(static_cast<uint32_t>(mask), 0u));
       const uint32_t take = pool_count < n_need ? pool_count : n_need;
-      if (need && rank < take) {
+      if (kScout) {
+        if (need && rank < take) {
+          const uint32_t sl = pool_count - 1u - rank;
+          const uint4 c0 = pool[sl * kChunks + 0], c1 = pool[sl * kChunks + 1], c2 = pool[sl * kChunks + 2];
+          o = v3(__uint_as_float(c0.x), __uint_as_float(c0.y), __uint_as_float(c0.z));
+          d = v3(__uint_as_float(c0.w), __uint_as_float(c1.x), __uint_as_float(c1.y));
+          rng = static_cast<uint64_t>(c1.z) | (static_cast<uint64_t>(c1.w) << 32);
+          q = c2.x; casts = c2.y; origin_slot = static_cast<int>(c2.z); scout_bound = c2.w;
+          alive = true;
+        }
+      } else if (need && rank < take) {
         const uint32_t sl = pool_count - 1u - rank;
         const uint4 c0 = pool[sl * kChunks + 0], c1 = pool[sl * kChunks + 1], c2 = pool[sl * kChunks + 2], c3 = pool[sl * kChunks + 3];
         o = v3(__uint_as_float(c0.x), __uint_as_float(c0.y), __uint_as_float(c0.z));
@@ -106,7 +123,14 @@
           const uint32_t gbase = claim_next;
           claim_next += n_new;
           const unsigned long long m_alive = __ballot(alive);
-          if (alive) {
+          if (kScout) {
+            if (alive) {
+              const uint32_t sl = __builtin_amdgcn_mbcnt_hi(static_cast<uint32_t>(m_alive >> 32), __builtin_amdgcn_mbcnt_lo(static_cast<uint32_t>(m_alive), 0u));
+              pool[sl * kChunks + 0] = make_uint4(__float_as_uint(o.x), __float_as_uint(o.y), __float_as_uint(o.z), __float_as_uint(d.x));
+              pool[sl * kChunks + 1] = make_uint4(__float_as_uint(d.y), __float_as_uint(d.z), static_cast<uint32_t>(rng), static_cast<uint32_t>(rng >> 32));
+              pool[sl * kChunks + 2] = make_uint4(q, casts, static_cast<uint32_t>(origin_slot), scout_bound);
+            }
+          } else if (alive) {
             const uint32_t sl = __builtin_amdgcn_mbcnt_hi(static_cast<uint32_t>(m_alive >> 32), __builtin_amdgcn_mbcnt_lo(static_cast<uint32_t>(m_alive), 0u));
             pool[sl * kChunks + 0] = make_uint4(__float_as_uint(o.x), __float_as_uint(o.y), __float_as_uint(o.z), __float_as_uint(d.x));
             pool[sl * kChunks + 1] = make_uint4(__float_as_uint(d.y), __float_as_uint(d.z), __float_as_uint(w.x), __float_as_uint(w.y));
@@ -138,8 +162,10 @@
               rng = XorShiftSeed(AMBER_ARG(cold, hashed_seed), px + py * eye.sensor.w, sample);
               float ew;
               bool near_edge = false;
-              GenerateEyeRay<kDivEye, SqrtModeOf(kSqrtMask, 4u)>(eye, px, py, rng, o, d, ew, origin_slot, &near_edge);
-              w = v3(ew, ew, ew);
+              GenerateEyeRay<kDivEye, SqrtModeOf(kSqrtMask, 4u), kScout>(eye, px, py, rng, o, d, ew, origin_slot, &near_edge);
+              if (kScout) {
+                scout_bound = (Abs(ew) >= amber_scout::kMinZ && Abs(ew) < __builtin_inff()) ? AMBER_ARG(cold, scout_bound0) : amber_scout::kSuspect;
+              } else w = v3(ew, ew, ew);
               const uint32_t* const pixel_mask = kTwoPhase ? AMBER_ARG(cold, pixel_mask) : nullptr;
               if (kTwoPhase && pixel_mask) {
                 premask = pixel_mask[plocal] | (origin_slot >= 0 ? 1u << origin_slot : 0u) | (near_edge ? AMBER_ARG(cold, scene.blade_mask) : 0u);
@@ -161,7 +187,7 @@
     bool emit = false;
     V3 meas = v3(0.f, 0.f, 0.f);
     if (alive) {
-      if (!kLight && carries) meas = ld3(AMBER_CARRIED());
+      if (!kLight && !kScout && carries) meas = ld3(AMBER_CARRIED());
       if (kLight) {
         const uint32_t plocal = Quotient(a.div_samples, q);
         const typename std::conditional<kPhotons, PhotonSink, SplatSink>::type sink = MakeLightSink<kPhotons>(a, a.path_offset + plocal, a.first_sample + (q - plocal * a.n_samples));
@@ -172,10 +198,14 @@
         sig_obj = Fnv32(sig_obj, static_cast<uint32_t>(b.object));
         if (b.object >= 0) sig_t = Fnv32(sig_t, __float_as_uint(b.t));
         if (!alive) AMBER_ARG(AMBER_COLD_OPEN(), sig)[q] = static_cast<unsigned long long>(sig_obj) | (static_cast<unsigned long long>(sig_t) << 32);
+      } else if (kScout) {
+        alive = PathStep<false, kEngine, false, kDivBasis, kDivHit, kSqrtMask, SINK_SCOUT>(sc, lds.objects, lds.stack, o, d, w, meas, rng, casts, origin_slot, nullptr AMBER_STAMP_ARG, nullptr, primary, premask, AMBER_PATH_BVH_STACK, &scout_bound);
+        emit = !alive && (((__float_as_uint(meas.x) | __float_as_uint(meas.y) | __float_as_uint(meas.z)) != 0u) || scout_bound > amber_scout::kLimit);
+        meas = v3(0.f, 0.f, 0.f);
       } else {
         alive = PathStep<false, kEngine, false, kDivBasis, kDivHit, kSqrtMask>(sc, lds.objects, lds.stack, o, d, w, meas, rng, casts, origin_slot, nullptr AMBER_STAMP_ARG, nullptr, primary, premask, AMBER_PATH_BVH_STACK);
       }
-      if (!kLight) {
+      if (!kLight && !kScout) {
         const bool nz = (__float_as_uint(meas.x) | __float_as_uint(meas.y) | __float_as_uint(meas.z)) != 0u;
         emit = !alive && nz;
         if (alive && nz) { float* c = AMBER_CARRIED(); c[0] = meas.x; c[1] = meas.y; c[2] = meas.z; carries = true; }
diff --git a/amber_amd/csrc/hip/pt_replay.inc b/amber_amd/csrc/hip/pt_replay.inc
--- /dev/null
+++ b/amber_amd/csrc/hip/pt_replay.inc
@@ -0,0 +1,28 @@
+template <int kEngine>
+__global__ void __launch_bounds__(256) replay_records_kernel(const RenderArgs a) {
+  const DevScene& sc = a.scene;
+  const EngineLds lds = StageEngineLds<kEngine, 1>(sc);
+  constexpr bool kDivBasis = (AMBER_SHARED_DIV_NORMALIZE & 1) != 0, kDivHit = (AMBER_SHARED_DIV_NORMALIZE & 2) != 0, kDivEye = (AMBER_SHARED_DIV_NORMALIZE & 4) != 0;
+  constexpr uint32_t kSqrtMask = static_cast<uint32_t>(AMBER_EXACT_SQRT);
+  const uint32_t claimed = *a.rec_count;
+  const uint32_t n = claimed < a.rec_capacity ? claimed : a.rec_capacity;
+  for (uint32_t i = blockIdx.x * 256u + threadIdx.x; i < n; i += gridDim.x * 256u) {
+    const uint32_t q = a.records[i].x;
+    if (q == AMBER_REC_UNUSED) continue;
+    const uint32_t plocal = Quotient(a.div_samples, q), sample = a.first_sample + (q - plocal * a.n_samples);
+    const uint32_t lrow = Quotient(a.div_width, plocal), px = plocal - lrow * sc.sensor.w;
+    const uint32_t py = FrameRow(a.row_begin, a.stripe_rows, a.stripe_period, a.div_stripe_rows, lrow);
+    uint64_t rng = XorShiftSeed(a.hashed_seed, px + py * sc.sensor.w, sample);
+    V3 o, d;
+    float ew;
+    int origin_slot = -1;
+    GenerateEyeRay<kDivEye, SqrtModeOf(kSqrtMask, 4u)>(sc, px, py, rng, o, d, ew, origin_slot);
+    V3 w = v3(ew, ew, ew), meas = v3(0.f, 0.f, 0.f);
+    uint32_t casts = 0;
+#ifdef AMBER_STAMPS
+    StampCtx stamp_store{}; StampCtx* stamp_ctx = &stamp_store;
+#endif
+    while (PathStep<false, kEngine, false, kDivBasis, kDivHit, kSqrtMask>(sc, lds.objects, lds.stack, o, d, w, meas, rng, casts, origin_slot, nullptr AMBER_STAMP_ARG)) {}
+    a.records[i] = make_uint4(q, __float_as_uint(meas.x), __float_as_uint(meas.y), __float_as_uint(meas.z));
+  }
+}
diff --git a/amber_amd/csrc/hip/scene_prep.h b/amber_amd/csrc/hip/scene_prep.h
--- a/amber_amd/csrc/hip/scene_prep.h
+++ b/amber_amd/csrc/hip/scene_prep.h
@@ -13,6 +13,7 @@
 #include "bvh_build.h"
 #include "filter_build.h"
 #include "ref_bvh_build.h"
+#include "scout_bound.h"
 
 namespace amber_prep {
 
@@ -172,6 +173,22 @@
     const double tol = min_edge > 0 ? std::max(1e-3, 64.0 * 5.9604644775390625e-08 * world_mag / min_edge) : 1.0;
     lens.edge_tol = static_cast<float>(std::min(1.0, tol));
   }
+}
+
+inline bool DecideScout(uint32_t engine, uint32_t hit_engine, uint32_t flags, const DevLens& lens, const std::vector<DevBlade>& blades, const std::vector<DevMaterial>& materials,
+                        float sensor_w, float sensor_h, uint32_t* bound0) {
+  *bound0 = 0;
+  if (engine == AMBER_ENGINE_WAVEFRONT || hit_engine != AMBER_ENGINE_TWO_PHASE || (flags & AMBER_PT_FLAG_NO_SCOUT)) return false;
+  for (const DevMaterial& m : materials)
+    for (float x : {m.rho[0], m.rho[1], m.rho[2], m.param, m.r0, m.aux0, m.aux1}) if (!std::isfinite(x)) return false;
+  std::vector<float> vertices;
+  for (const DevBlade& bl : blades) for (const float* v : {bl.v0, bl.v1, bl.v2}) vertices.insert(vertices.end(), v, v + 3);
+  amber_scout::LensFacts f{};
+  f.kind = lens.kind; f.local_ = lens.local_; f.global_ = lens.global_; f.origin = lens.origin;
+  f.sensor_distance = lens.sensor_distance; f.focus_distance = lens.focus_distance; f.p_area = lens.p_area; f.size_over_area = lens.size_over_area;
+  f.inv_scene_area = lens.inv_scene_area; f.sensor_w = sensor_w; f.sensor_h = sensor_h;
+  f.blade_vertices = vertices.data(); f.n_vertices = static_cast<uint32_t>(vertices.size() / 3u);
+  return amber_scout::EyeWeightBound(f, bound0);
 }
 
 inline void DeriveLensOfState(const SceneState& st, const AmberFlatThinLens& L, const AmberFlatObject* blade_records,
diff --git a/amber_amd/csrc/hip/scout_bound.h b/amber_amd/csrc/hip/scout_bound.h
--- /dev/null
+++ b/amber_amd/csrc/hip/scout_bound.h
@@ -0,0 +1,74 @@
+#pragma once
+
+#include <cmath>
+#include <cstdint>
+
+#if defined(__HIPCC__)
+#define AMBER_SCOUT_HD __host__ __device__
+#else
+#define AMBER_SCOUT_HD
+#endif
+
+namespace amber_scout {
+
+constexpr uint32_t kLimit = 126u * 16u;
+constexpr uint32_t kSuspect = 0x40000000u;
+constexpr float kMinZ = 0.015625f;
+constexpr float kMinGap = 9.094947017729282e-13f;
+
+AMBER_SCOUT_HD inline uint32_t BounceBound(uint32_t bound, uint32_t sx_bits, uint32_t sy_bits, uint32_t sz_bits, uint32_t p_bits) {
+  const uint32_t ax = sx_bits & 0x7fffffffu, ay = sy_bits & 0x7fffffffu, az = sz_bits & 0x7fffffffu;
+  uint32_t a = ax > ay ? ax : ay;
+  a = a > az ? a : az;
+  uint32_t inc = ((a >> 23) - (p_bits >> 23) + 1u) * 16u;
+  if (p_bits == 0x3f700000u && a <= 0x3f800000u) inc = 2u;
+  if (a <= p_bits) inc = 0u;
+  bound += inc;
+  if (a >= 0x7f800000u || p_bits < 0x00800000u || p_bits >= 0x7f800000u) bound = kSuspect;
+  return bound < kSuspect ? bound : kSuspect;
+}
+
+struct LensFacts {
+  uint32_t kind;
+  const float* local_; const float* global_;
+  const float* origin;
+  float sensor_distance, focus_distance, p_area, size_over_area, inv_scene_area;
+  float sensor_w, sensor_h;
+  const float* blade_vertices; uint32_t n_vertices;
+};
+
+inline bool EyeWeightBound(const LensFacts& f, uint32_t* bound0) {
+  const double kHi = 1048576.0, kLo = 1.0 / 1048576.0;
+  auto in_range = [&](double x) { return std::isfinite(x) && std::fabs(x) >= kLo && std::fabs(x) <= kHi; };
+  auto positive = [&](double x) { return x >= 0x1p-60 && x <= 0x1p60; };
+  if (f.kind > 1u) return false;
+  if (!in_range(f.sensor_distance) || !in_range(f.sensor_w) || !in_range(f.sensor_h) || !(f.sensor_w > 0) || !(f.sensor_h > 0)) return false;
+  for (int c = 0; c < 3; c++) if (!(std::fabs(double(f.origin[c])) <= kHi)) return false;
+  for (const float* m : {f.local_, f.global_})
+    for (int i = 0; i < 3; i++)
+      for (int j = 0; j < 3; j++) {
+        double rr = 0, cc = 0;
+        for (int k = 0; k < 3; k++) { rr += double(m[3 * i + k]) * m[3 * j + k]; cc += double(m[3 * k + i]) * m[3 * k + j]; }
+        const double want = i == j ? 1.0 : 0.0;
+        if (!(std::fabs(rr - want) <= 1e-3) || !(std::fabs(cc - want) <= 1e-3)) return false;
+      }
+  const double sd2 = double(f.sensor_distance) * f.sensor_distance;
+  double log2_bound;
+  if (f.kind == 1u) {
+    if (!positive(f.inv_scene_area)) return false;
+    log2_bound = std::log2(1.03 / (sd2 * f.inv_scene_area));
+  } else {
+    if (!in_range(f.focus_distance) || !positive(f.p_area) || !positive(f.size_over_area)) return false;
+    for (uint32_t k = 0; k < 3u * f.n_vertices; k++) if (!(std::fabs(double(f.blade_vertices[k])) <= kHi)) return false;
+    const double factor_max = std::pow(1.0001 / double(kMinZ), 4.0), pdf_min = double(f.size_over_area) * sd2 / std::pow(1.01, 4.0);
+    log2_bound = std::log2(factor_max / double(f.p_area) / pdf_min);
+  }
+  if (!std::isfinite(log2_bound)) return false;
+  const double sixteenths = std::ceil(16.0 * (log2_bound + 1.0));
+  const double b = sixteenths < 0 ? 0.0 : sixteenths;
+  if (b > double(kLimit) - 16.0 * 16.0) return false;
+  *bound0 = static_cast<uint32_t>(b);
+  return true;
+}
+
+}
diff --git a/include/amber_hip.h b/include/amber_hip.h
--- a/include/amber_hip.h
+++ b/include/amber_hip.h
@@ -94,7 +94,8 @@
   AMBER_PT_FLAG_NULL_STREAM = 1u,
   AMBER_PT_FLAG_BVH_POOL = 2u,
   AMBER_PT_FLAG_BVH_ITEMS = 4u,
-  AMBER_PT_FLAG_DEVICE_BUILD = 8u
+  AMBER_PT_FLAG_DEVICE_BUILD = 8u,
+  AMBER_PT_FLAG_NO_SCOUT = 16u
 };
 
 enum {
diff --git a/include/amber_hip_lab.h b/include/amber_hip_lab.h
--- a/include/amber_hip_lab.h
+++ b/include/amber_hip_lab.h
@@ -36,6 +36,7 @@
 typedef struct { uint32_t n_launches, n_repeats, rec_count, flag_words_set, flags_dirty; } AmberAccumulateInfo;
 int amber_hip_kat_accumulate(amber_hip_pt*, uint32_t n_samples, const uint32_t* q , const float* rgb , uint32_t n_items,
                              uint32_t n_waves, uint32_t rec_capacity, uint64_t rays, AmberAccumulateInfo* info);
+int amber_hip_kat_scout_flags(amber_hip_pt*, uint32_t first_sample, uint32_t n_samples, uint32_t* out_flags, uint64_t n_words, uint32_t* out_scouts, uint32_t* out_bound0);
 int amber_hip_kat_lt_stage_ms(amber_hip_pt*, double* sort_ms, double* sum_ms);
 int amber_hip_kat_photon_stage_ms(amber_hip_pt*, double* trace_ms, double* sort_ms, double* gather_ms);
 int amber_hip_kat_math(int device, int mode, uint32_t n, const float* x, float* out);
```

After: 51610, median of 6. 7.3% higher.
